# scheckmedia/centernet-uda

Measured on AMD Instinct MI355X. Metric: images/sec CenterNet DLA-34 512x512 UDA step (entropy minimisation), higher is better.
Workload: dtype f32; 1 GPU; configs[2]: DLA-34 + DCNv2, 512x512, per-GPU batch 16 source + 16 target, uda=entropy_minimization, Adam(lr 5e-5), random-init weights; global_batch=16, parallelism=dp1

## Files before the change

centernet-uda_amd/backends/dla.py:

```python
import logging
import math
import os
import warnings

import torch
from torch import nn

from hip_runtime import nn as hnn
from hip_runtime import ops
from hip_runtime.fanout import fork
from libs.DCNv2.dcn_v2 import DCN

log = logging.getLogger(__name__)
PRETRAINED_FILE = 'dla34-ba72cf86.pth'

BN_MOMENTUM = 0.1
DLA34_LEVELS = (1, 1, 1, 2, 2, 1)
DLA34_CHANNELS = (16, 32, 64, 128, 256, 512)


def _bn(c):
    return hnn.BatchNorm2d(c, momentum=BN_MOMENTUM)


_FOLD_GEN = [0]


def _fold_stamp(module):
    import hip_runtime as hr
    if not hasattr(module, '_fold_token'):
        module._fold_token = hr.PackToken()
    _FOLD_GEN[0] += 1
    module._fold_gen = _FOLD_GEN[0]


def _folded(conv_weight, conv_bias, bn):
    with torch.no_grad():
        scale = bn.weight / torch.sqrt(bn.running_var + bn.eps)
        w = (conv_weight * scale.view(-1, 1, 1, 1)).contiguous()
        b = bn.bias - bn.running_mean * scale
        if conv_bias is not None:
            b = b + conv_bias * scale
        return w, b.contiguous()


_FOLDED_INFERENCE = False


class folded_inference:

    def __enter__(self):
        global _FOLDED_INFERENCE
        self.prev, _FOLDED_INFERENCE = _FOLDED_INFERENCE, True

    def __exit__(self, *exc):
        global _FOLDED_INFERENCE
        _FOLDED_INFERENCE = self.prev


def _use_folded(module):
    return (_FOLDED_INFERENCE and getattr(module, '_fold', None) is not None and not module.training
            and not torch.is_grad_enabled())


def fold_batchnorm(model):
    n = 0
    for m in model.modules():
        if hasattr(m, 'fold_batchnorm_'):
            m.fold_batchnorm_()
            n += 1
    return n


def unfold_batchnorm(model):
    for m in model.modules():
        if hasattr(m, 'fold_batchnorm_'):
            m._fold = None


def _conv(cin, cout, k, stride=1):
    return hnn.Conv2d(cin, cout, k, stride=stride, padding=k // 2, bias=False, emit_stats=True)


def _norm_on_load_ok(cin, cout, k):
    try:
        import hip_runtime as hr
        return bool(hr.lib().cnuda_conv2d_norm_input_supported(1, cin, 64, 64, cout, k, k, 1, 1, k // 2, k // 2))
    except Exception:
        return False


class ConvBnRelu(nn.Sequential):

    _fold = None

    def __init__(self, cin, cout, k, stride=1):
        super().__init__(_conv(cin, cout, k, stride), _bn(cout))

    def fold_batchnorm_(self):
        self._fold = _folded(self[0].weight, self[0].bias, self[1])
        _fold_stamp(self)

    def forward(self, x):
        if _use_folded(self):
            return ops.conv2d_infer(x, *self._fold, self[0].stride, self[0].padding, 0.0, None, self._fold_token,
                                    self._fold_gen)
        return self[1](self[0](x), relu=True)


class ConvBn(nn.Sequential):
    _fold = None

    def __init__(self, cin, cout):
        super().__init__(_conv(cin, cout, 1), _bn(cout))

    def fold_batchnorm_(self):
        self._fold = _folded(self[0].weight, self[0].bias, self[1])
        _fold_stamp(self)

    def forward(self, x):
        if _use_folded(self):
            return ops.conv2d_infer(x, *self._fold, self[0].stride, self[0].padding, -1.0, None, self._fold_token,
                                    self._fold_gen)
        return self[1](self[0](x))


class BasicBlock(nn.Module):
    def __init__(self, cin, cout, stride=1):
        super().__init__()
        self.conv1, self.bn1 = _conv(cin, cout, 3, stride), _bn(cout)
        self.conv2, self.bn2 = _conv(cout, cout, 3), _bn(cout)

    _fold = None

    def fold_batchnorm_(self):
        import hip_runtime as hr
        self._fold = _folded(self.conv1.weight, None, self.bn1) + _folded(self.conv2.weight, None, self.bn2)
        _fold_stamp(self)
        if not hasattr(self, '_fold_token2'):
            self._fold_token2 = hr.PackToken()

    def forward(self, x, residual=None):
        if _use_folded(self):
            w1, b1, w2, b2 = self._fold
            y = ops.conv2d_infer(x, w1, b1, self.conv1.stride, self.conv1.padding, 0.0, None, self._fold_token,
                                 self._fold_gen)
            return ops.conv2d_infer(y, w2, b2, 1, 1, 0.0, x if residual is None else residual, self._fold_token2,
                                    self._fold_gen)
        if residual is None or residual is x:
            x, residual = fork(x, 2)
        y = self.bn1(self.conv1(x), relu=True)
        return self.bn2(self.conv2(y), residual=residual, relu=True)


CAT_FREE_ROOT = os.environ.get('CNUDA_CAT_FREE_ROOT', '1') != '0'


class Root(nn.Module):
    def __init__(self, cin, cout):
        super().__init__()
        self.conv, self.bn = _conv(cin, cout, 1), _bn(cout)

    _fold = None

    def fold_batchnorm_(self):
        self._fold = _folded(self.conv.weight, None, self.bn)
        _fold_stamp(self)

    def forward(self, *xs):
        if _use_folded(self):
            y = ops.conv1x1_cat_infer(xs, *self._fold, 0.0, self._fold_token, self._fold_gen) if CAT_FREE_ROOT else None
            return y if y is not None else ops.conv2d_infer(ops.cat_channels(xs), *self._fold, 1, 0, 0.0, None,
                                                            self._fold_token, self._fold_gen)
        y = ops.conv1x1_cat(xs, self.conv.weight, self.conv._pack_token, emit_stats=self.conv.emit_stats and self.training) \
            if CAT_FREE_ROOT and self.conv.kernel_size == (1, 1) and self.conv.bias is None else None
        if y is None:
            y = self.conv(ops.cat_channels(xs))
        return self.bn(y, relu=True)


class Tree(nn.Module):

    def __init__(self, levels, cin, cout, stride=1, level_root=False, root_dim=0):
        super().__init__()
        self.levels, self.level_root = levels, level_root
        root_dim = root_dim or 2 * cout
        if level_root:
            root_dim += cin
        if levels == 1:
            self.tree1 = BasicBlock(cin, cout, stride)
            self.tree2 = BasicBlock(cout, cout, 1)
            self.root = Root(root_dim, cout)
        else:
            self.tree1 = Tree(levels - 1, cin, cout, stride)
            self.tree2 = Tree(levels - 1, cout, cout, root_dim=root_dim + cout)
        self.downsample = hnn.MaxPool2d(stride) if stride > 1 else None
        self.project = ConvBn(cin, cout) if cin != cout else None

    def forward(self, x, children=None):
        children = [] if children is None else children
        if self.downsample is not None:
            x_pool, x = fork(x, 2)
            bottom = self.downsample(x_pool)
            takers = int(self.project is not None or self.levels == 1) + int(self.level_root)
            bs = list(fork(bottom, takers)) if takers > 1 else [bottom]
            residual = self.project(bs.pop()) if self.project is not None else (bs.pop() if self.levels == 1 else None)
            if self.level_root:
                children.append(bs.pop())
        else:
            takers = 1 + int(self.project is not None) + int(self.level_root)
            xs = list(fork(x, takers)) if takers > 1 else [x]
            x = xs.pop()
            residual = self.project(xs.pop()) if self.project is not None else x
            if self.level_root:
                children.append(xs.pop())
        if self.levels == 1:
            x1 = self.tree1(x, residual)
            x1_next, x1_root = fork(x1, 2)
            x2 = self.tree2(x1_next)
            return self.root(x2, x1_root, *children)
        x1 = self.tree1(x)
        x1_next, x1_root = fork(x1, 2)
        children.append(x1_root)
        return self.tree2(x1_next, children=children)


class DLA(nn.Module):
    def __init__(self, levels=DLA34_LEVELS, channels=DLA34_CHANNELS):
        super().__init__()
        c = self.channels = list(channels)
        self.base_layer = ConvBnRelu(3, c[0], 7)
        self.level0 = ConvBnRelu(c[0], c[0], 3)
        self.base_layer[1].defer_apply = _norm_on_load_ok(c[0], c[0], 3)
# ... 292 lines not shown
```

centernet-uda_amd/csrc/conv.hip:

```cpp
#include <stdlib.h>

#include <type_traits>
#include <algorithm>
#include "igemm.cuh"
#include "hconv.cuh"
#include "hwgrad.cuh"
#include "igemm_host.h"

namespace cnuda {
namespace {

struct ConvGeom {
    int B, C, H, W, Co, kh, kw, sh, sw, ph, pw, Ho, Wo;
};

struct ConvFwdParams {
    ConvGeom g;
    const float *x, *bias;
    float* y;
    float act_slope;
    const float* residual;
};
struct ConvFwdStatsParams : ConvFwdParams {
    float* stats;
    int stats_mp;
};

struct ConvFwdSigParams : ConvFwdParams {
    int sig_from;
};
__device__ __forceinline__ float conv_row_sigmoid(float v) { return 1.0f / (1.0f + expf(-v)); }

template <bool FAST>
struct ConvFwdLoader {
    using Params = ConvFwdParams;
    static const char* name() { return FAST ? "ConvFwdLoader<true>" : "ConvFwdLoader<false>"; }
    static constexpr bool kHasSideOutput = false;
    const ConvGeom& g;
    const float* x_b;
    int iy0, ix0;
    bool valid;
    int ck0 = 0, ctap = 0, cc0 = 0, cr = 0, cs = 0;
    __device__ __forceinline__ void seek(int k0) {
        while (ck0 < k0) {
            ck0 += IG_BK;
            cc0 += IG_BK;
            if (cc0 >= g.C) { cc0 -= g.C; ++ctap; if (++cs == g.kw) { cs = 0; ++cr; } }
        }
    }
    __device__ ConvFwdLoader(const Params& p, long long n, bool n_valid) : g(p.g), valid(n_valid) {
        const int HoWo = g.Ho * g.Wo;
        const int nn = n_valid ? (int)n : 0;
        const int b = nn / HoWo, pp = nn - b * HoWo;
        const int oy = pp / g.Wo, ox = pp - oy * g.Wo;
        iy0 = oy * g.sh - g.ph;
        ix0 = ox * g.sw - g.pw;
        x_b = p.x + (size_t)b * g.C * g.H * g.W;
    }
    __device__ __forceinline__ void load(int k0, int ksub, float (&v)[8]) {
        const int HW = g.H * g.W, K = g.kh * g.kw * g.C;
        if (FAST) {
            seek(k0);
            const int c0 = cc0 + ksub;
            const int iy = iy0 + cr, ix = ix0 + cs;
            const bool ok = valid && k0 < K && iy >= 0 && iy < g.H && ix >= 0 && ix < g.W;
            const float* ptr = x_b + (size_t)c0 * HW + (ok ? iy * g.W + ix : 0);
#pragma unroll
            for (int j = 0; j < 8; ++j) v[j] = ok ? ptr[(size_t)(2 * j) * HW] : 0.0f;
        } else {
#pragma unroll
            for (int j = 0; j < 8; ++j) {
                const int k = k0 + ksub + 2 * j;
                float val = 0.0f;
                if (valid && k < K) {
                    const int tap = k / g.C, c = k - tap * g.C;
                    const int r = tap / g.kw, s = tap - r * g.kw;
                    const int iy = iy0 + r, ix = ix0 + s;
                    if (iy >= 0 && iy < g.H && ix >= 0 && ix < g.W) val = x_b[(size_t)c * HW + iy * g.W + ix];
                }
                v[j] = val;
            }
        }
    }
    struct Out {
        float* base;
        const float* res;
        int HoWo;
        __device__ Out(const Params& p, long long n) {
            HoWo = p.g.Ho * p.g.Wo;
            const int ni = (int)n, b = ni / HoWo, pp = ni - b * HoWo;
            base = p.y + (size_t)b * p.g.Co * HoWo + pp;
            res = p.residual ? p.residual + (size_t)b * p.g.Co * HoWo + pp : nullptr;
        }
        __device__ __forceinline__ void store(const Params& p, int m, float v) {
            if (p.bias) v += p.bias[m];
            if (res) v += res[(size_t)m * HoWo];
            if (p.act_slope >= 0.0f && v < 0.0f) v *= p.act_slope;
            base[(size_t)m * HoWo] = v;
        }
        static constexpr bool kVec4 = true;
        __device__ static bool vec4_ok(const Params& p) { return ((p.g.Ho * p.g.Wo) & 3) == 0; }
        __device__ __forceinline__ void store4(const Params& p, int m, f32x4 v) {
            if (p.bias) v += p.bias[m];
            if (res) v += *reinterpret_cast<const f32x4*>(res + (size_t)m * HoWo);
            if (p.act_slope >= 0.0f) {
#pragma unroll
                for (int e = 0; e < 4; ++e) if (v[e] < 0.0f) v[e] *= p.act_slope;
            }
            *reinterpret_cast<f32x4*>(base + (size_t)m * HoWo) = v;
        }
    };
};

struct ConvFwdBufLoader {
    using Params = ConvFwdParams;
    static const char* name() { return "ConvFwdBufLoader"; }
    static constexpr bool kHasSideOutput = false;
    const ConvGeom& g;
    buf_rsrc rs;
    unsigned pix_off;
    unsigned tap_ok;
    int ck0 = 0, ctap = 0, cc0 = 0, cr = 0, cs = 0;
    __device__ __forceinline__ void seek(int k0) {
        while (ck0 < k0) {
            ck0 += IG_BK;
            cc0 += IG_BK;
            if (cc0 >= g.C) { cc0 -= g.C; ++ctap; if (++cs == g.kw) { cs = 0; ++cr; } }
        }
    }
    __device__ ConvFwdBufLoader(const Params& p, long long n, bool n_valid) : g(p.g) {
        const int HoWo = g.Ho * g.Wo;
        const int nn = n_valid ? (int)n : 0;
        const int b = nn / HoWo, pp = nn - b * HoWo;
        const int oy = pp / g.Wo, ox = pp - oy * g.Wo;
        const int iy0 = oy * g.sh - g.ph, ix0 = ox * g.sw - g.pw;
        rs = ig_make_rsrc(p.x, (unsigned)((size_t)g.B * g.C * g.H * g.W * sizeof(float)));
        pix_off = (unsigned)(((b * g.C * g.H + iy0) * g.W + ix0) * (int)sizeof(float));
        tap_ok = 0;
        if (n_valid) {
            for (int r = 0; r < g.kh; ++r)
                for (int s = 0; s < g.kw; ++s) {
                    const int iy = iy0 + r, ix = ix0 + s;
                    if (iy >= 0 && iy < g.H && ix >= 0 && ix < g.W) tap_ok |= 1u << (r * g.kw + s);
                }
        }
    }
    __device__ __forceinline__ void load(int k0, int ksub, float (&v)[8]) {
        const int HW = g.H * g.W;
        seek(k0);
        const int tap = ctap < 32 ? ctap : 31;
        const bool in_k = k0 < g.kh * g.kw * g.C;
        const unsigned voff = (in_k && ((tap_ok >> tap) & 1u)) ? pix_off + (unsigned)((cr * g.W + cs) * (int)sizeof(float))
                                                                : IG_BUF_OOB;
        const int c0 = cc0 + __builtin_amdgcn_readfirstlane(ksub);
#pragma unroll
        for (int j = 0; j < 8; ++j) v[j] = ig_buf_load(rs, voff, (unsigned)((c0 + 2 * j) * HW) * (unsigned)sizeof(float));
    }
    using Out = ConvFwdLoader<true>::Out;
};

struct ConvFwdBufSigLoader : ConvFwdBufLoader {
    using Params = ConvFwdSigParams;
    static const char* name() { return "ConvFwdBufSigLoader"; }
    __device__ ConvFwdBufSigLoader(const Params& p, long long n, bool n_valid) : ConvFwdBufLoader(p, n, n_valid) {}
    struct Out : ConvFwdLoader<true>::Out {
        __device__ Out(const Params& p, long long n) : ConvFwdLoader<true>::Out(p, n) {}
        __device__ __forceinline__ void store(const Params& p, int m, float v) {
            if (p.bias) v += p.bias[m];
            if (m >= p.sig_from) v = conv_row_sigmoid(v);
            base[(size_t)m * HoWo] = v;
        }
        __device__ __forceinline__ void store4(const Params& p, int m, f32x4 v) {
            if (p.bias) v += p.bias[m];
            if (m >= p.sig_from) {
#pragma unroll
                for (int e = 0; e < 4; ++e) v[e] = conv_row_sigmoid(v[e]);
            }
            *reinterpret_cast<f32x4*>(base + (size_t)m * HoWo) = v;
        }
    };
};

struct ConvFwdBufQuadLoader : ConvFwdBufLoader {
    static const char* name() { return "ConvFwdBufQuadLoader"; }
    __device__ ConvFwdBufQuadLoader(const Params& p, long long n, bool n_valid) : ConvFwdBufLoader(p, n, n_valid) {}
    struct Out {
        float* base;
        size_t quad_stride;
        __device__ Out(const Params& p, long long n) {
            const int HoWo = p.g.Ho * p.g.Wo;
            const int ni = (int)n, b = ni / HoWo, pp = ni - b * HoWo;
            base = p.y + (size_t)b * p.g.Co * HoWo + (size_t)pp * 4;
            quad_stride = (size_t)HoWo * 4;
        }
        __device__ __forceinline__ void store(const Params&, int m, float v) { base[(size_t)(m >> 2) * quad_stride + (m & 3)] = v; }
        static constexpr bool kVec4 = false;
        __device__ static bool vec4_ok(const Params&) { return false; }
        static constexpr bool kQuads = true;
        __device__ __forceinline__ void store_quad(const Params&, int m, f32x4 v) {
            *reinterpret_cast<f32x4*>(base + (size_t)(m >> 2) * quad_stride) = v;
        }
    };
};

struct ConvFwdBufStatsLoader : ConvFwdBufLoader {
    using Params = ConvFwdStatsParams;
    static const char* name() { return "ConvFwdBufStatsLoader"; }
    __device__ ConvFwdBufStatsLoader(const Params& p, long long n, bool n_valid) : ConvFwdBufLoader(p, n, n_valid) {}
};

constexpr int CAT_MAX = 4;
struct ConvCat {
    const float* x[CAT_MAX];
    int c[CAT_MAX];
    int k0[CAT_MAX + 1];
    int n;
};
struct ConvFwdCatParams : ConvFwdStatsParams {
    ConvCat cat;
};
struct ConvFwdCatLoader {
    using Params = ConvFwdCatParams;
    static const char* name() { return "ConvFwdCatLoader"; }
    static constexpr bool kHasSideOutput = false;
    const Params& p;
    unsigned pix;
    int b;
    bool valid;
    int ck0 = 0, src = 0, cc0 = 0;
    __device__ ConvFwdCatLoader(const Params& pp, long long n, bool n_valid) : p(pp), valid(n_valid) {
        const int HW = p.g.H * p.g.W;
        const int nn = n_valid ? (int)n : 0;
        b = nn / HW;
        pix = (unsigned)(nn - b * HW) * 4u;
    }
    __device__ __forceinline__ void load(int k0, int ksub, float (&v)[8]) {
        const int HW = p.g.H * p.g.W;
        while (ck0 < k0) {
            ck0 += IG_BK;
            cc0 += IG_BK;
            if (src < p.cat.n && cc0 >= p.cat.c[src]) { cc0 = 0; ++src; }
        }
        const bool in_k = src < p.cat.n;
        const int s = in_k ? src : 0, cs = p.cat.c[s];
        const buf_rsrc rs = ig_make_rsrc(p.cat.x[s], (unsigned)((size_t)p.g.B * cs * HW * sizeof(float)));
        const unsigned voff = (valid && in_k) ? (unsigned)(b * cs * HW) * 4u + pix : IG_BUF_OOB;
        const int c0 = cc0 + __builtin_amdgcn_readfirstlane(ksub);
#pragma unroll
        for (int j = 0; j < 8; ++j) v[j] = ig_buf_load(rs, voff, (unsigned)((c0 + 2 * j) * HW) * (unsigned)sizeof(float));
    }
    using Out = ConvFwdLoader<true>::Out;
};

struct ConvDgradParams {
    ConvGeom g;
    const float* gy;
    float* gx;
    int cop;
    const float* add = nullptr;
    const float* add2 = nullptr;
};
struct ConvDgradLoader {
    using Params = ConvDgradParams;
    static const char* name() { return "ConvDgradLoader"; }
    static constexpr bool kHasSideOutput = false;
    const ConvGeom& g;
    const float* gy_b;
// ... 217 lines not shown
            const int ni = (int)n, b = ni / HcWc, q = ni - b * HcWc;
            const int qy = q / p.Wc, qx = q - qy * p.Wc;
            const size_t o = (size_t)b * p.g.C * HW + (size_t)(p.py + qy * p.g.sh) * p.g.W + p.px + qx * p.g.sw;
            base = p.gx + o;
            addb = p.add ? p.add + o : nullptr;
            addc = p.add2 ? p.add2 + o : nullptr;
        }
        __device__ __forceinline__ void store(const Params&, int m, float v) {
            if (addb) v += addb[(size_t)m * HW];
            if (addc) v += addc[(size_t)m * HW];
            base[(size_t)m * HW] = v;
        }
        static constexpr bool kVec4 = false;
        __device__ static bool vec4_ok(const Params&) { return false; }
        __device__ __forceinline__ void store4(const Params&, int, f32x4) {}
    };
};

struct ConvDgradClassBufLoader {
    using Params = ConvDgradClassParams;
    static const char* name() { return "ConvDgradClassBufLoader"; }
    static constexpr bool kHasSideOutput = false;
    const Params& p;
    buf_rsrc rs;
    unsigned pix_off, tap_ok;
    int ck0 = 0, cti = 0, co0 = 0;
    __device__ ConvDgradClassBufLoader(const Params& pp, long long n, bool n_valid) : p(pp) {
        const ConvGeom& g = p.g;
        const int HcWc = p.Hc * p.Wc;
        const int nn = n_valid ? (int)n : 0;
        const int b = nn / HcWc, q = nn - b * HcWc;
        const int qy = q / p.Wc, qx = q - qy * p.Wc;
        rs = ig_make_rsrc(p.gy, (unsigned)((size_t)g.B * g.Co * g.Ho * g.Wo * sizeof(float)));
        pix_off = (unsigned)(((b * g.Co * g.Ho + qy) * g.Wo + qx) * (int)sizeof(float));
        tap_ok = 0;
        if (n_valid) {
            for (int t = 0; t < p.ntaps; ++t) {
                const int oy = qy + p.tap_dy[t], ox = qx + p.tap_dx[t];
                if (oy >= 0 && oy < g.Ho && ox >= 0 && ox < g.Wo) tap_ok |= 1u << t;
            }
        }
    }
    __device__ __forceinline__ void load(int k0, int ksub, float (&v)[8]) {
        const ConvGeom& g = p.g;
        const int HoWo = g.Ho * g.Wo;
        while (ck0 < k0) {
            ck0 += IG_BK;
            co0 += IG_BK;
            if (co0 >= g.Co) { co0 -= g.Co; ++cti; }
        }
        const int ti = cti < p.ntaps ? cti : 0;
        const int tapoff = p.tap_dy[ti] * g.Wo + p.tap_dx[ti];
        const unsigned voff = (cti < p.ntaps && ((tap_ok >> ti) & 1u)) ? pix_off + (unsigned)(tapoff * (int)sizeof(float))
                                                                        : IG_BUF_OOB;
        const int o0 = co0 + __builtin_amdgcn_readfirstlane(ksub);
#pragma unroll
        for (int j = 0; j < 8; ++j) v[j] = ig_buf_load(rs, voff, (unsigned)((o0 + 2 * j) * HoWo) * (unsigned)sizeof(float));
    }
    using Out = ConvDgradClassLoader::Out;
};

constexpr int MAX_CLASSES = 4;
struct ConvDgradClassSet {
    ConvDgradClassParams cls[MAX_CLASSES];
    const float* A[MAX_CLASSES];
    int Kp[MAX_CLASSES];
};
template <int BM>
__global__ __launch_bounds__(2 * IG_THREADS, (BM == 128 ? 2 : 1)) void igemm_fwd_ws_classes_kernel(
    ConvDgradClassSet s, int Mp, int M, long long N, int n_tiles, int m_tiles) {
    const int c = blockIdx.y;
    igemm_fwd_ws_body<BM, ConvDgradClassBufLoader, IG_KC>(s.cls[c], s.A[c], Mp, s.Kp[c], M, N, n_tiles, m_tiles);
}
template <int BM>
__global__ __launch_bounds__(IG_THREADS, (BM == 128 ? 3 : 1)) void igemm_fwd_classes_kernel(
    ConvDgradClassSet s, int Mp, int M, long long N, int n_tiles, int m_tiles) {
    const int c = blockIdx.y;
    igemm_fwd_body<BM, ConvDgradClassBufLoader>(s.cls[c], s.A[c], Mp, s.Kp[c], M, N, n_tiles, m_tiles);
}

struct ConvWParams {
    ConvGeom g;
    const float *x, *gy;
};
template <int MODE>
struct ConvWLoader {
    using Params = ConvWParams;
    static const char* name() { return MODE == 2 ? "ConvWLoader<2>" : (MODE == 1 ? "ConvWLoader<1>" : "ConvWLoader<0>"); }
    const Params& p;
    IgPixelCursor c;
    __device__ ConvWLoader(const Params& pp, long long n, long long n_end) : p(pp) {
        c.init(n, n_end, p.g.Ho * p.g.Wo, p.g.Wo);
    }
    __device__ __forceinline__ void advance() { c.advance(p.g.Ho * p.g.Wo, p.g.Wo); }
    template <int NV, int STEP>
    __device__ __forceinline__ void load_g(int m0, int msub, float (&v)[NV]) {
        const ConvGeom& g = p.g;
        const int HoWo = g.Ho * g.Wo;
        const float* base = p.gy + (size_t)c.b_ * g.Co * HoWo + c.pp_;
#pragma unroll
        for (int i = 0; i < NV; ++i) {
            const int m = m0 + msub + STEP * i;
            v[i] = (c.valid_ && m < g.Co) ? base[(size_t)m * HoWo] : 0.0f;
        }
    }
    template <int NV, int STEP>
    __device__ __forceinline__ void load_b(int j0, int jsub, float (&v)[NV]) {
        const ConvGeom& g = p.g;
        const int HW = g.H * g.W, K = g.kh * g.kw * g.C;
        const int iy0 = c.oy_ * g.sh - g.ph, ix0 = c.ox_ * g.sw - g.pw;
        const float* x_b = p.x + (size_t)c.b_ * g.C * HW;
        if (MODE == 2) {
            constexpr int PER = 64 / STEP;
#pragma unroll
            for (int h = 0; h < NV / PER; ++h) {
                const int jg = j0 + 64 * h;
                const int tap = jg / g.C, c0 = jg - tap * g.C + jsub;
                const int r = tap / g.kw, s = tap - r * g.kw;
                const int iy = iy0 + r, ix = ix0 + s;
                const bool ok1 = c.valid_ && jg < K && iy >= 0 && iy < g.H && ix >= 0 && ix < g.W;
                const float* ptr = x_b + (size_t)c0 * HW + (ok1 ? iy * g.W + ix : 0);
#pragma unroll
                for (int i = 0; i < PER; ++i) v[PER * h + i] = ok1 ? ptr[(size_t)(STEP * i) * HW] : 0.0f;
            }
            return;
        }
        int cur = -1, off = 0;
        bool ok = false;
#pragma unroll
        for (int i = 0; i < NV; ++i) {
            const int k = j0 + jsub + STEP * i;
            float val = 0.0f;
            if (c.valid_ && k < K) {
                const int tap = k / g.C, ch = k - tap * g.C;
                if (tap != cur) {
                    const int r = tap / g.kw, s = tap - r * g.kw;
                    const int iy = iy0 + r, ix = ix0 + s;
                    ok = iy >= 0 && iy < g.H && ix >= 0 && ix < g.W;
                    off = iy * g.W + ix;
                    cur = tap;
                }
                if (ok) val = x_b[(size_t)ch * HW + off];
            }
            v[i] = val;
        }
    }
};

struct ConvWBufLoader {
    using Params = ConvWParams;
    static const char* name() { return "ConvWBufLoader"; }
    const Params& p;
    buf_rsrc rg, rx;
    IgPixelCursor c;
    unsigned gimg, ximg;
    __device__ ConvWBufLoader(const Params& pp, long long n, long long n_end) : p(pp) {
        const ConvGeom& g = p.g;
        rg = ig_make_rsrc(p.gy, (unsigned)((size_t)g.B * g.Co * g.Ho * g.Wo * sizeof(float)));
        rx = ig_make_rsrc(p.x, (unsigned)((size_t)g.B * g.C * g.H * g.W * sizeof(float)));
        c.init(n, n_end, g.Ho * g.Wo, g.Wo);
        gimg = (unsigned)(c.b_ * g.Co * g.Ho * g.Wo) * 4u;
        ximg = (unsigned)(c.b_ * g.C * g.H * g.W) * 4u;
    }
    __device__ __forceinline__ void advance() {
        const ConvGeom& g = p.g;
        c.advance(g.Ho * g.Wo, g.Wo);
        if (c.crossed_) {
            gimg += (unsigned)(c.crossed_ * g.Co * g.Ho * g.Wo) * 4u;
            ximg += (unsigned)(c.crossed_ * g.C * g.H * g.W) * 4u;
        }
    }
    template <int NV, int STEP>
    __device__ __forceinline__ void load_g(int m0, int msub, float (&v)[NV]) {
        ig_buf_rows<NV, STEP>(rg, c, gimg, p.g.Ho * p.g.Wo, m0, msub, v);
    }
    template <int NV, int STEP>
    __device__ __forceinline__ void load_b(int j0, int jsub, float (&v)[NV]) {
        const ConvGeom& g = p.g;
        const int HW = g.H * g.W, K = g.kh * g.kw * g.C;
        const int iy0 = ig_mad24(c.oy_, g.sh, -g.ph), ix0 = ig_mad24(c.ox_, g.sw, -g.pw);
        const unsigned corner = ximg + (unsigned)(ig_mad24(jsub, HW, ig_mad24(iy0, g.W, ix0))) * 4u;
        constexpr int PER = 64 / STEP;
#pragma unroll
        for (int h = 0; h < NV / PER; ++h) {
            const int jg = j0 + 64 * h;
            const int tap = jg / g.C, c0 = jg - tap * g.C;
            const int r = tap / g.kw, s = tap - r * g.kw;
            const int iy = iy0 + r, ix = ix0 + s;
            const bool ok = c.valid_ && jg < K && (unsigned)iy < (unsigned)g.H && (unsigned)ix < (unsigned)g.W;
            const unsigned voff = ok ? corner + (unsigned)((r * g.W + s) * (int)sizeof(float)) : IG_BUF_OOB;
#pragma unroll
            for (int i = 0; i < PER; ++i)
                v[PER * h + i] = ig_buf_load(rx, voff, (unsigned)((c0 + STEP * i) * HW) * (unsigned)sizeof(float));
        }
    }
};

struct ConvWBufLoaderC8 : ConvWBufLoader {
    static const char* name() { return "ConvWBufLoaderC8"; }
    __device__ ConvWBufLoaderC8(const Params& pp, long long n, long long n_end) : ConvWBufLoader(pp, n, n_end) {}
    template <int NV, int STEP>
    __device__ __forceinline__ void load_b(int j0, int jsub, float (&v)[NV]) {
        static_assert(STEP == 8, "eight row phases: a phase's channels stay inside one tap when 8 | C");
        const ConvGeom& g = p.g;
        const int HW = g.H * g.W, K = g.kh * g.kw * g.C;
        const int iy0 = ig_mad24(c.oy_, g.sh, -g.ph), ix0 = ig_mad24(c.ox_, g.sw, -g.pw);
        const unsigned corner = ximg + (unsigned)(ig_mad24(jsub, HW, ig_mad24(iy0, g.W, ix0))) * 4u;
#pragma unroll
        for (int i = 0; i < NV; ++i) {
            const int jg = j0 + STEP * i;
            const int tap = jg / g.C, c0 = jg - tap * g.C;
            const int r = tap / g.kw, s = tap - r * g.kw;
            const int iy = iy0 + r, ix = ix0 + s;
            const bool ok = c.valid_ && jg < K && (unsigned)iy < (unsigned)g.H && (unsigned)ix < (unsigned)g.W;
            const unsigned voff = ok ? corner + (unsigned)((r * g.W + s) * (int)sizeof(float)) : IG_BUF_OOB;
            v[i] = ig_buf_load(rx, voff, (unsigned)(c0 * HW) * (unsigned)sizeof(float));
        }
    }
};

struct ConvWCatParams : ConvWParams {
    ConvCat cat;
};
struct ConvWCatLoader {
    using Params = ConvWCatParams;
    static const char* name() { return "ConvWCatLoader"; }
    const Params& p;
    buf_rsrc rg;
    IgPixelCursor c;
    unsigned gimg;
    __device__ ConvWCatLoader(const Params& pp, long long n, long long n_end) : p(pp) {
        const ConvGeom& g = p.g;
        rg = ig_make_rsrc(p.gy, (unsigned)((size_t)g.B * g.Co * g.Ho * g.Wo * sizeof(float)));
        c.init(n, n_end, g.Ho * g.Wo, g.Wo);
        gimg = (unsigned)(c.b_ * g.Co * g.Ho * g.Wo) * 4u;
    }
    __device__ __forceinline__ void advance() {
        const ConvGeom& g = p.g;
        c.advance(g.Ho * g.Wo, g.Wo);
        if (c.crossed_) gimg += (unsigned)(c.crossed_ * g.Co * g.Ho * g.Wo) * 4u;
    }
    template <int NV, int STEP>
    __device__ __forceinline__ void load_g(int m0, int msub, float (&v)[NV]) {
        ig_buf_rows<NV, STEP>(rg, c, gimg, p.g.Ho * p.g.Wo, m0, msub, v);
    }
    template <int NV, int STEP>
    __device__ __forceinline__ void load_b(int j0, int jsub, float (&v)[NV]) {
        const ConvGeom& g = p.g;
        const int HW = g.H * g.W;
        constexpr int PER = 64 / STEP;
#pragma unroll
        for (int h = 0; h < NV / PER; ++h) {
            const int jg = j0 + 64 * h;
            int s = 0;
#pragma unroll
            for (int i = 1; i < CAT_MAX; ++i) s += (i < p.cat.n && jg >= p.cat.k0[i]) ? 1 : 0;
            const int cs = p.cat.c[s], c0 = jg - p.cat.k0[s];
            const buf_rsrc rx = ig_make_rsrc(p.cat.x[s], (unsigned)((size_t)g.B * cs * HW * sizeof(float)));
            const bool ok = c.valid_ && jg < g.C;
            const unsigned voff = ok ? (unsigned)(ig_mad24(c.b_, cs, jsub) * HW + c.pp_) * 4u : IG_BUF_OOB;
#pragma unroll
            for (int i = 0; i < PER; ++i)
                v[PER * h + i] = ig_buf_load(rx, voff, (unsigned)((c0 + STEP * i) * HW) * (unsigned)sizeof(float));
        }
    }
};

int fill_geom(ConvGeom& g, int B, int C, int H, int W, int Co, int kh, int kw, int sh, int sw, int ph, int pw,
              const char* who) {
    CNUDA_REQUIRE(B > 0 && C > 0 && H > 0 && W > 0 && Co > 0, "%s: empty tensor", who);
    CNUDA_REQUIRE(kh > 0 && kw > 0 && sh > 0 && sw > 0 && ph >= 0 && pw >= 0, "%s: bad kernel geometry", who);
    g = ConvGeom{B, C, H, W, Co, kh, kw, sh, sw, ph, pw, (H + 2 * ph - kh) / sh + 1, (W + 2 * pw - kw) / sw + 1};
    CNUDA_REQUIRE(H + 2 * ph >= kh && W + 2 * pw >= kw && g.Ho > 0 && g.Wo > 0, "%s: kernel larger than padded input",
                  who);
    return 0;
}

bool wgrad_buffer_ok(const ConvGeom& g) {
    return buffer_addressing() && (size_t)g.B * g.C * g.H * g.W * sizeof(float) < IG_BUF_OOB &&
           (size_t)g.B * g.Co * g.Ho * g.Wo * sizeof(float) < IG_BUF_OOB && (long long)g.H * g.W < (1 << 23) &&
           (long long)g.Ho * g.Wo < (1 << 23);
}
// ... 123 lines not shown
    const long long z = wgrad_splits(tiles, q.wbm, q.wbj, (q.Nf + WG_BP - 1) / WG_BP);
    q.pix_per_split = ((q.Nf + z - 1) / z + WG_BP - 1) / WG_BP * WG_BP;
    q.Z = (int)((q.Nf + q.pix_per_split - 1) / q.pix_per_split);
    q.hw = hwgrad_ok(g);
    q.hw_s2 = !q.hw && hwgrad_s2_ok(g);
    q.hw_tiles = q.hw_tiles_per_split = 0;
    if (q.hw || q.hw_s2) {
        q.hw_tiles = q.hw ? g.B * hwgrad_tiles_y(g) * (g.W / halo_tile_width(g.W)) : g.B * g.Ho * (round_up(g.Wo, HS_BN) / HS_BN);
        const int groups = (g.C / 16) * (q.hw_s2 ? (g.Co + 31) / 32 : 1);
        int zz = std::max(1, 512 / groups);
        if (zz > q.hw_tiles) zz = q.hw_tiles;
        q.hw_tiles_per_split = (q.hw_tiles + zz - 1) / zz;
        q.Z = (q.hw_tiles + q.hw_tiles_per_split - 1) / q.hw_tiles_per_split;
    }
    q.fwd_bytes = carve_bytes(ig_a_bytes(q.Kpf, q.Mpf), 1) + carve_bytes(splitk_slab_bytes(q.skf, g.Co, q.Nf), 1) + 256;
    q.dgrad_bytes = carve_bytes(ig_a_bytes(q.Kpd, q.Mpd), 1) + carve_bytes(splitk_slab_bytes(q.skd, g.C, q.Nd), 1) + 256;
    if (g.sh > 1 || g.sw > 1) {
        const long long Nc = q.Nd / (g.sh * g.sw);
        const int Kpc = round_up(ceil_div(g.kh, g.sh) * ceil_div(g.kw, g.sw) * g.Co, IG_KC);
        const SplitK sc = pick_splitk(g.C, Nc, Kpc);
        const int mp = round_up(g.C, sc.on() ? sc.bm : 32);
        const size_t need = (size_t)g.sh * g.sw * carve_bytes(ig_a_bytes(Kpc, std::max(round_up(g.C, 128), std::max(mp, q.Mpd))), 1) +
                            carve_bytes(splitk_slab_bytes(sc, g.C, Nc), 1) + 256;
        if (need > q.dgrad_bytes) q.dgrad_bytes = need;
    }
    q.wgrad_bytes = carve_bytes((size_t)q.Z * q.Mpw * q.Jp, 4) +
                    carve_bytes(std::max((size_t)g.Co * g.B, (size_t)q.Z * q.Mpw), 4) + 256;

    q.fwd_gemm = q.skf.on() ? FwdPath::BufSplitK
               : hconv_ok(g, g.C, q.bmf) ? FwdPath::Halo
               : q.fwd_buf ? FwdPath::Buf
               : g.C % IG_BK == 0 ? FwdPath::PtrFast : FwdPath::Ptr;
    q.fwd = smallc_supported(g.C, g.Co, g.kh, g.kw, g.sh, g.sw) ? FwdPath::SmallC : q.fwd_gemm;

    if (g.C == 16 && g.kh == 3 && g.kw == 3 && g.sh == 2 && g.sw == 2 && g.ph == 1 && g.pw == 1 && g.Co <= 256 &&
        matrix_mode() == 0 && (size_t)g.Co * 144 * sizeof(float) <= ig_a_bytes(q.Kpd, q.Mpd)) {
        q.dgrad_gemm = DgradPath::S2C16;
    } else if ((g.sh > 1 || g.sw > 1) && g.H % g.sh == 0 && g.W % g.sw == 0 && g.Co % IG_BK == 0 &&
               ceil_div(g.kh, g.sh) * ceil_div(g.kw, g.sw) <= 9) {
        const long long Nc = (long long)g.B * (g.H / g.sh) * (g.W / g.sw);
        bool any_split = false;
        for (int py = 0; py < g.sh && q.dgrad_buf && !any_split; ++py)
            for (int px = 0; px < g.sw && !any_split; ++px) {
                int ntaps = 0;
                for (int r = 0; r < g.kh; ++r)
                    for (int t = 0; t < g.kw; ++t) ntaps += class_tap(g, py, px, r, t);
                any_split = pick_splitk(g.C, Nc, class_kp(ntaps, g.Co)).on();
            }
        q.dgrad_gemm = (q.dgrad_buf && !any_split && g.sh * g.sw <= MAX_CLASSES && matrix_mode() == 0) ? DgradPath::Classes
                                                                                                    : DgradPath::ClassLoop;
    } else {
        q.dgrad_gemm = q.skd.on() ? DgradPath::BufSplitK
                     : hconv_ok(g, g.Co, q.bmd) ? DgradPath::Halo
                     : (q.dgrad_buf && g.sh == 1 && g.sw == 1) ? DgradPath::Buf : DgradPath::Ptr;
    }
    q.dgrad = (g.sh == 1 && g.sw == 1 && smallc_supported(g.Co, g.C, g.kh, g.kw, 1, 1) && g.kh - 1 - g.ph >= 0 && g.kw - 1 - g.pw >= 0)
                  ? DgradPath::SmallC : q.dgrad_gemm;

    const bool fast = g.C % 64 == 0;
    q.wgrad = smallc_supported(g.C, g.Co, g.kh, g.kw, g.sh, g.sw) ? WgradPath::SmallC
            : q.hw_s2 ? WgradPath::HaloS2
            : q.hw ? WgradPath::Halo
            : (!fast && g.C % 8 == 0 && wbuf && (q.wbm == 32 || (q.wbm == 64 && q.wbj == 64))) ? WgradPath::BufC8
            : (fast && wbuf) ? WgradPath::Buf
            : (fast && wave_specialised() && q.wbm == 64) ? WgradPath::PtrFastWs
            : fast ? WgradPath::PtrFast : WgradPath::Ptr;
    q.wgrad_ws = wave_specialised() && q.wbm >= 64 && (q.wgrad == WgradPath::Buf || q.wgrad == WgradPath::PtrFastWs);
    q.max_bytes = std::max(q.fwd_bytes, std::max(q.dgrad_bytes, q.wgrad_bytes));
    if (q.fwd == FwdPath::SmallC || smallc_supported(g.Co, g.C, g.kh, g.kw, g.sh, g.sw))
        q.max_bytes = std::max(q.max_bytes, smallc_workspace_bytes(g.B, g.C, g.H, g.W, g.Co, g.kh, g.kw, g.sh, g.ph, g.pw) +
                                                carve_bytes((size_t)g.Co * g.B, 4));
    return q;
}

int plan_stats_block(const ConvGeom& g, const ConvPlan& q, int* rows, int* blocks_per_image) {
    if (blocks_per_image) *blocks_per_image = 0;
    if (q.fwd == FwdPath::SmallC)
        return smallc_stats_blocks(g.B, g.C, g.H, g.W, g.Co, g.kh, g.kw, g.sh, g.ph, g.pw, blocks_per_image, rows);
    if (q.fwd != FwdPath::Buf || ((g.Ho * g.Wo) & 3) != 0 || matrix_mode() != 0) return 0;
    if (rows) *rows = q.Mpf;
    return q.bmf == 32 ? 32 : 64;
}

struct HconvFwd {
    using Params = ConvFwdParams;
    using Out = ConvFwdLoader<true>::Out;
    static const char* name() { return "fwd"; }
};
struct HconvFwdSig {
    using Params = ConvFwdSigParams;
    using Out = ConvFwdBufSigLoader::Out;
    static const char* name() { return "fwd, row sigmoid"; }
};
struct HconvDgrad {
    using Params = ConvDgradParams;
    using Out = ConvDgradLoader::Out;
    static const char* name() { return "dgrad"; }
};
template <int BM, int BN, class Ad>
bool hconv_launch_one(const typename Ad::Params& p, const float* src, const float* A, int Mp, int Kp, int M, long long N,
                      int m_tiles, const HaloGeom& hg, hipStream_t st) {
    const size_t lds = hconv_lds_bytes(hg, BM);
    if (!raise_dynamic_lds(reinterpret_cast<const void*>(&hconv_kernel<BM, BN, Ad>), lds)) return false;
    const int n_tiles = (int)(N / ((long long)hg.H * hg.W)) * hg.tiles_y * hg.tiles_x;
    CNUDA_LAUNCH((hconv_kernel<BM, BN, Ad>), dim3(n_tiles * m_tiles), dim3(IG_THREADS), lds, st, p, src, A, Mp, Kp, M, N,
                 n_tiles, m_tiles, hg);
    return true;
}
template <class Ad>
int launch_hconv(int bm, const typename Ad::Params& p, const float* src, int kc, const ConvGeom& g, const float* A, int Mp,
                 int Kp, int M, long long N, hipStream_t st, const char* who) {
    CNUDA_REQUIRE(N < (1ll << 31) - 256, "%s: more than 2^31 pixels per call", who);
    const int m_tiles = Mp / bm;
    const HaloGeom hg2 = make_halo_geom(kc, g.H, g.W, 256);
    const bool wide = bm <= 64 && hg2.TW >= 32 && g.H % hg2.TR == 0 && hg2.cells <= HC_MAXCELLS * IG_THREADS &&
                      (N / 256) * m_tiles >= 1024;
    const HaloGeom hg = wide ? hg2 : make_halo_geom(kc, g.H, g.W, 128);
    ProfScope prof(st);
    prof.name("hconv_kernel<%d, %d, %s>", bm, wide ? 256 : 128, Ad::name());
    bool ok = false;
    CNUDA_REQUIRE((with_tiles<Tile<128, 128>, Tile<64, 256>, Tile<64, 128>, Tile<32, 256>, Tile<32, 128>>(
                      bm, wide ? 256 : 128, [&](auto BM, auto BN) {
                          ok = hconv_launch_one<BM(), BN(), Ad>(p, src, A, Mp, Kp, M, N, m_tiles, hg, st);
                      })),
                  "%s: no hconv_kernel instance for a %d-row tile", who, bm);
    if (!ok) return CNUDA_ERR_INVALID_ARGUMENT;
    return check_launch(who);
}

struct DgradS2Params {
    const float *gy, *wt;
    float* gx;
    const float *add, *add2;
    int B, Co, H, W, Ho, Wo, QH, QW;
};
__global__ __launch_bounds__(256) void dgrad_s2_c16_pack_kernel(const float* __restrict__ w, float* __restrict__ wt, int Co) {
    const int i = blockIdx.x * 256 + threadIdx.x;
    if (i < Co * 144) {
        const int c = i & 15, t = (i >> 4) % 9, o = i / 144;
        wt[i] = w[(o * 16 + c) * 9 + t];
    }
}
__global__ __launch_bounds__(256) void dgrad_s2_c16_kernel(DgradS2Params p) {
    const int qx = blockIdx.x * 64 + (threadIdx.x & 63);
    const int qy = blockIdx.y * 4 + (threadIdx.x >> 6);
    const int b = blockIdx.z;
    if (qy >= p.QH) return;
    const int HoWo = p.Ho * p.Wo, HW = p.H * p.W;
    const bool x0 = qx < p.Wo, x1 = qx + 1 < p.Wo, y0 = qy < p.Ho, y1 = qy + 1 < p.Ho;
    const float* g00 = p.gy + (size_t)b * p.Co * HoWo + (size_t)(y0 ? qy : 0) * p.Wo + (x0 ? qx : 0);
    const int d01 = x1 ? 1 : 0, d10 = y1 ? p.Wo : 0;
    float acc[4][16];
#pragma unroll
    for (int q = 0; q < 4; ++q)
#pragma unroll
        for (int c = 0; c < 16; ++c) acc[q][c] = 0.0f;
    for (int o = 0; o < p.Co; ++o) {
        const float* gp = g00 + (size_t)o * HoWo;
        float a = gp[0], bb = gp[d01], cc = gp[d10], dd = gp[d10 + d01];
        if (!(x0 && y0)) a = 0.0f;
        if (!(x1 && y0)) bb = 0.0f;
        if (!(x0 && y1)) cc = 0.0f;
        if (!(x1 && y1)) dd = 0.0f;
        const float* wo = p.wt + (size_t)o * 144;
#pragma unroll
        for (int c = 0; c < 16; ++c) {
// ... 38 lines not shown
template <class Loader>
int launch_fwd(int bm, const typename Loader::Params& p, const float* A, int Mp, int Kp, int M, long long N,
               hipStream_t st, const char* who, const SplitK& sk = SplitK(), float* slab = nullptr) {
    CNUDA_REQUIRE(N < (1ll << 31) - IG_BN, "%s: more than 2^31 pixels per call", who);
    const int n_tiles = ceil_div(N, IG_BN), m_tiles = Mp / bm;
    const dim3 grid(n_tiles * m_tiles), block(IG_THREADS), block2(2 * IG_THREADS);
    const bool ws = matrix_mode() == 0 && wave_specialised() && bm >= 64;
    bool found;
    ProfScope prof(st);
    if constexpr (SplitKLoader<Loader>::value) {
        if (sk.on()) {
            CNUDA_REQUIRE(slab && bm == sk.bm && matrix_mode() == 0, "%s: split-K plan without its slabs", who);
            prof.name(ws ? "igemm_fwd_ws_splitk_kernel<%d, %s> x %d + reduce" : "igemm_fwd_splitk_kernel<%d, %s> x %d + reduce",
                      bm, Loader::name(), sk.z);
            const dim3 gridz(n_tiles * m_tiles, sk.z);
            if (ws)
                found = with_tile<64, 128>(bm, [&](auto BM) {
                    CNUDA_LAUNCH((igemm_fwd_ws_splitk_kernel<BM(), Loader>), gridz, block2, 0, st, p, A, Mp, Kp, M, N, n_tiles, m_tiles, slab, sk.split_k);
                });
            else
                found = with_tile<32, 64, 128>(bm, [&](auto BM) {
                    CNUDA_LAUNCH((igemm_fwd_splitk_kernel<BM(), Loader>), gridz, block, 0, st, p, A, Mp, Kp, M, N, n_tiles, m_tiles, slab, sk.split_k);
                });
            CNUDA_REQUIRE(found, "%s: no split-K kernel instance for a %d-row tile", who, bm);
            CNUDA_LAUNCH((splitk_reduce_kernel<Loader>), dim3(ceil_div(N, 256), ceil_div(M, SK_ROWS)), dim3(256), 0, st, p, slab, sk.z,
                         Mp, (long long)n_tiles * IG_BN, M, N);
            return check_launch(who);
        }
    }
    CNUDA_REQUIRE(!sk.on(), "%s: split-K plan for a loader without split-K kernels", who);
    if constexpr (std::is_same<Loader, ConvFwdBufLoader>::value || std::is_same<Loader, ConvFwdBufStatsLoader>::value ||
                  std::is_same<Loader, ConvFwdLoader<true>>::value || std::is_same<Loader, ConvFwdBufQuadLoader>::value) {
        static const bool shortk = !(getenv("CNUDA_SHORTK") && getenv("CNUDA_SHORTK")[0] == '0');
        if (shortk && matrix_mode() == 0 && bm == 128 && Kp <= 64 && m_tiles >= 2) {
            prof.name("igemm_fwd_shortk_kernel<128, %s, 64>", Loader::name());
            CNUDA_LAUNCH((igemm_fwd_shortk_kernel<128, Loader, 64>), dim3(n_tiles), block, 0, st, p, A, Mp, Kp, M, N,
                               n_tiles, m_tiles);
            return check_launch(who);
        }
    }
    prof.name(matrix_mode() == 1 ? "igemm_fwd_kernel<%d, %s> [split bf16 x3]"
                                 : (ws ? "igemm_fwd_ws_kernel<%d, %s>" : "igemm_fwd_kernel<%d, %s>"), bm, Loader::name());
    if (matrix_mode() == 1) {
        float* A3 = const_cast<float*>(A) + (size_t)Kp * Mp;
        CNUDA_LAUNCH(split_a_kernel, dim3(stream_grid((long long)(Kp / 16) * 2 * Mp, 256)), dim3(256), 0, st, A,
                           reinterpret_cast<u32x4*>(A3), Kp, Mp);
        found = with_tile<32, 64, 128>(bm, [&](auto BM) {
            CNUDA_LAUNCH((igemm_fwd_kernel<BM(), Loader, true>), grid, block, 0, st, p, A3, Mp, Kp, M, N, n_tiles, m_tiles);
        });
    } else if (ws) {
        found = with_tile<64, 128>(bm, [&](auto BM) {
            CNUDA_LAUNCH((igemm_fwd_ws_kernel<BM(), Loader>), grid, block2, 0, st, p, A, Mp, Kp, M, N, n_tiles, m_tiles);
        });
    } else {
        found = with_tile<32, 64, 128>(bm, [&](auto BM) {
            CNUDA_LAUNCH((igemm_fwd_kernel<BM(), Loader>), grid, block, 0, st, p, A, Mp, Kp, M, N, n_tiles, m_tiles);
        });
    }
    CNUDA_REQUIRE(found, "%s: no igemm_fwd kernel instance for a %d-row tile", who, bm);
    return check_launch(who);
}

template <class Loader, bool WS, class... Tiles, class P>
bool launch_wgrad(const ConvPlan& q, const P& p, float* slabs, float* bsl, hipStream_t st) {
    const dim3 grid(q.Jp / q.wbj, q.Mpw / q.wbm, q.Z), blk((WS ? 2 : 1) * IG_THREADS);
    return with_tiles<Tiles...>(q.wbm, q.wbj, [&](auto BM, auto BJ) {
        if constexpr (WS)
            CNUDA_LAUNCH((igemm_wgrad_ws_kernel<Loader, BM(), BJ()>), grid, blk, 0, st, p, slabs, q.Mpw, q.Jp, q.Nf, q.pix_per_split, bsl);
        else
            CNUDA_LAUNCH((igemm_wgrad_kernel<Loader, BM(), BJ()>), grid, blk, 0, st, p, slabs, q.Mpw, q.Jp, q.Nf, q.pix_per_split, bsl);
    });
}
template <class Loader>
bool launch_wgrad_buf(const ConvPlan& q, const typename Loader::Params& p, float* slabs, float* bsl, hipStream_t st) {
    return q.wgrad_ws ? launch_wgrad<Loader, true, Tile<128, 128>, Tile<128, 64>, Tile<64, 128>, Tile<64, 64>>(q, p, slabs, bsl, st)
                      : launch_wgrad<Loader, false, Tile<128, 128>, Tile<128, 64>, Tile<64, 128>, Tile<64, 64>, Tile<32, 128>>(q, p, slabs, bsl, st);
}

}
}

using namespace cnuda;


extern "C" int cnuda_conv_set_splitk_policy(int max_tiles) {
    const int prev = g_splitk_max_tiles;
    g_splitk_max_tiles = max_tiles < 0 ? 128 : max_tiles;
    return prev;
}

extern "C" int cnuda_conv_set_halo_policy(int level, int min_tiles) {
    if (level >= 0) g_hconv_level = level;
    if (min_tiles >= 1) g_hconv_min_tiles = min_tiles;
    return g_hconv_level | (g_hconv_min_tiles << 8);
}

extern "C" size_t cnuda_conv2d_workspace_bytes(int B, int C, int H, int W, int Cout, int kh, int kw, int sh, int sw,
                                               int ph, int pw) {
    ConvGeom g;
    if (fill_geom(g, B, C, H, W, Cout, kh, kw, sh, sw, ph, pw, "cnuda_conv2d_workspace_bytes")) return 0;
    return make_plan(g).max_bytes;
}

extern "C" int cnuda_conv2d_forward(const float* x, const float* weight, const float* bias, float* y, int B, int C,
                                    int H, int W, int Cout, int kh, int kw, int sh, int sw, int ph, int pw, float act_slope,
                                    void* workspace, size_t workspace_bytes, cnuda_stream_t stream) {
    return cnuda_conv2d_forward_res(x, weight, bias, nullptr, y, B, C, H, W, Cout, kh, kw, sh, sw, ph, pw, act_slope,
                                    workspace, workspace_bytes, stream);
}

extern "C" int cnuda_conv2d_stats_block(int B, int C, int H, int W, int Cout, int kh, int kw, int sh, int sw, int ph,
                                        int pw, int* rows, int* blocks_per_image) {
    ConvGeom g;
    if (fill_geom(g, B, C, H, W, Cout, kh, kw, sh, sw, ph, pw, "cnuda_conv2d_stats_block")) return 0;
    return plan_stats_block(g, make_plan(g), rows, blocks_per_image);
}

extern "C" int cnuda_conv2d_forward_res(const float* x, const float* weight, const float* bias, const float* residual,
                                        float* y, int B, int C, int H, int W, int Cout, int kh, int kw, int sh, int sw,
                                        int ph, int pw, float act_slope, void* workspace, size_t workspace_bytes,
                                        cnuda_stream_t stream) {
    return cnuda_conv2d_forward_stats(x, weight, bias, residual, y, nullptr, B, C, H, W, Cout, kh, kw, sh, sw, ph, pw, act_slope,
                                      workspace, workspace_bytes, stream);
}

extern "C" int cnuda_conv2d_forward_stats(const float* x, const float* weight, const float* bias, const float* residual,
                                          float* y, float* stats, int B, int C, int H, int W, int Cout, int kh, int kw,
                                          int sh, int sw, int ph, int pw, float act_slope, void* workspace,
                                          size_t workspace_bytes, cnuda_stream_t stream) {
    CNUDA_REQUIRE(x && weight && y, "cnuda_conv2d_forward: null pointer");
    ConvGeom g;
    if (int rc = fill_geom(g, B, C, H, W, Cout, kh, kw, sh, sw, ph, pw, "cnuda_conv2d_forward")) return rc;
    const ConvPlan q = make_plan(g);
    CNUDA_REQUIRE(!stats || (!residual && act_slope < 0.0f && plan_stats_block(g, q, nullptr, nullptr) != 0),
                  "cnuda_conv2d_forward_stats: no statistics for this call (cnuda_conv2d_stats_block says which)");
    const FwdPath path = residual ? q.fwd_gemm : q.fwd;
    if (path == FwdPath::SmallC)
        return smallc_forward(x, weight, bias, y, B, C, H, W, Cout, kh, kw, sh, ph, pw, act_slope, 0, workspace,
                              workspace_bytes, (hipStream_t)stream, stats);
    CNUDA_REQUIRE(workspace && workspace_bytes >= q.fwd_bytes, "cnuda_conv2d_forward: workspace too small");
    hipStream_t st = (hipStream_t)stream;
    Carver cv(workspace, workspace_bytes);
    ConvFwdParams p{g, x, bias, y, act_slope, residual};
    const float* A = launch_pack(weight, reinterpret_cast<float*>(cv.take<char>(ig_a_bytes(q.Kpf, q.Mpf))), ig_a_bytes(q.Kpf, q.Mpf),
                                 Cout, C, q.T, path == FwdPath::Halo ? PACK_HALO_FWD : PACK_FWD, q.Kpf, q.Mpf, 0, st);
    switch (path) {
        case FwdPath::Halo:
            return launch_hconv<HconvFwd>(q.bmf, p, x, C, g, A, q.Mpf, q.Kpf, Cout, q.Nf, st, "cnuda_conv2d_forward");
        case FwdPath::BufSplitK: {
            float* slab = reinterpret_cast<float*>(cv.take<char>(splitk_slab_bytes(q.skf, Cout, q.Nf)));
            return launch_fwd<ConvFwdBufLoader>(q.bmf, p, A, q.Mpf, q.Kpf, Cout, q.Nf, st, "cnuda_conv2d_forward", q.skf, slab);
        }
        case FwdPath::Buf:
            if (stats) {
                ConvFwdStatsParams ps;
                static_cast<ConvFwdParams&>(ps) = p;
                ps.stats = stats;
                ps.stats_mp = q.Mpf;
                return launch_fwd<ConvFwdBufStatsLoader>(q.bmf, ps, A, q.Mpf, q.Kpf, Cout, q.Nf, st, "cnuda_conv2d_forward_stats");
            }
            return launch_fwd<ConvFwdBufLoader>(q.bmf, p, A, q.Mpf, q.Kpf, Cout, q.Nf, st, "cnuda_conv2d_forward");
        case FwdPath::PtrFast:
            return launch_fwd<ConvFwdLoader<true>>(q.bmf, p, A, q.Mpf, q.Kpf, Cout, q.Nf, st, "cnuda_conv2d_forward");
        default:
            return launch_fwd<ConvFwdLoader<false>>(q.bmf, p, A, q.Mpf, q.Kpf, Cout, q.Nf, st, "cnuda_conv2d_forward");
    }
}

namespace {
int fill_cat(ConvCat& cat, const float* const* xs, const int* cs, int n, const char* who) {
    CNUDA_REQUIRE(xs && cs && n >= 2 && n <= CAT_MAX, "%s: 2 .. %d sources", who, CAT_MAX);
    int k = 0;
    for (int i = 0; i < CAT_MAX; ++i) {
        cat.x[i] = i < n ? xs[i] : nullptr;
        cat.c[i] = i < n ? cs[i] : 0;
        cat.k0[i] = k;
        if (i < n) {
            CNUDA_REQUIRE(xs[i] && cs[i] > 0 && cs[i] % 64 == 0, "%s: source %d: null or not a multiple of 64 channels", who, i);
            k += cs[i];
        }
    }
    cat.k0[CAT_MAX] = k;
    for (int i = n; i < CAT_MAX; ++i) cat.k0[i] = k;
    cat.n = n;
    return 0;
}
int cat_channels(const int* cs, int n) {
    int k = 0;
    for (int i = 0; i < n; ++i) k += cs[i];
    return k;
}
}

extern "C" int cnuda_conv2d_cat_supported(const int* cs, int n, int B, int H, int W, int Cout) {
    if (!cs || n < 2 || n > CAT_MAX || matrix_mode() != 0) return 0;
    for (int i = 0; i < n; ++i)
        if (cs[i] <= 0 || cs[i] % 64 != 0) return 0;
    const int C = cat_channels(cs, n);
    ConvGeom g;
    if (fill_geom(g, B, C, H, W, Cout, 1, 1, 1, 1, 0, 0, "cnuda_conv2d_cat_supported")) return 0;
    const ConvPlan q = make_plan(g);
    return q.fwd == FwdPath::Buf && q.dgrad == DgradPath::Buf && q.wgrad == WgradPath::Buf && ((H * W) & 3) == 0;
}

extern "C" int cnuda_conv2d_cat_forward(const float* const* xs, const int* cs, int n, const float* weight, const float* bias,
                                        float* y, float* stats, float act_slope, int B, int H, int W, int Cout,
                                        void* workspace, size_t workspace_bytes, cnuda_stream_t stream) {
    CNUDA_REQUIRE(weight && y, "cnuda_conv2d_cat_forward: null pointer");
    CNUDA_REQUIRE(!stats || act_slope < 0.0f, "cnuda_conv2d_cat_forward: statistics are those of the plain convolution");
    CNUDA_REQUIRE(cnuda_conv2d_cat_supported(cs, n, B, H, W, Cout), "cnuda_conv2d_cat_forward: unsupported (cnuda_conv2d_cat_supported)");
    ConvFwdCatParams p;
    if (int rc = fill_cat(p.cat, xs, cs, n, "cnuda_conv2d_cat_forward")) return rc;
    const int C = p.cat.k0[CAT_MAX];
    ConvGeom g;
    if (int rc = fill_geom(g, B, C, H, W, Cout, 1, 1, 1, 1, 0, 0, "cnuda_conv2d_cat_forward")) return rc;
    const ConvPlan q = make_plan(g);
    CNUDA_REQUIRE(workspace && workspace_bytes >= q.fwd_bytes, "cnuda_conv2d_cat_forward: workspace too small");
    hipStream_t st = (hipStream_t)stream;
    Carver cv(workspace, workspace_bytes);
    static_cast<ConvFwdParams&>(p) = ConvFwdParams{g, nullptr, bias, y, act_slope, nullptr};
    p.stats = stats;
    p.stats_mp = q.Mpf;
    const float* A = launch_pack(weight, reinterpret_cast<float*>(cv.take<char>(ig_a_bytes(q.Kpf, q.Mpf))),
                                 ig_a_bytes(q.Kpf, q.Mpf), Cout, C, q.T, PACK_FWD, q.Kpf, q.Mpf, 0, st);
    return launch_fwd<ConvFwdCatLoader>(q.bmf, p, A, q.Mpf, q.Kpf, Cout, q.Nf, st, "cnuda_conv2d_cat_forward");
}
// ... 39 lines not shown
    ConvGeom g;
    if (int rc = fill_geom(g, B, C, H, W, Cout, 1, 1, 1, 1, 0, 0, "cnuda_conv2d_cat_backward_weight")) return rc;
    const ConvPlan q = make_plan(g);
    CNUDA_REQUIRE(workspace && workspace_bytes >= q.wgrad_bytes, "cnuda_conv2d_cat_backward_weight: workspace too small");
    hipStream_t st = (hipStream_t)stream;
    Carver cv(workspace, workspace_bytes);
    float* slabs = cv.take<float>((size_t)q.Z * q.Mpw * q.Jp);
    static_cast<ConvWParams&>(p) = ConvWParams{g, nullptr, grad_y};
    {
        ProfScope prof(st);
        prof.name(q.wgrad_ws ? "igemm_wgrad_ws_kernel<ConvWCatLoader, %d, %d>" : "igemm_wgrad_kernel<ConvWCatLoader, %d, %d>",
                  q.wbm, q.wbj);
        CNUDA_REQUIRE(launch_wgrad_buf<ConvWCatLoader>(q, p, slabs, nullptr, st),
                      "cnuda_conv2d_cat_backward_weight: no kernel instance for a %d x %d tile", q.wbm, q.wbj);
    }
    if (int rc = check_launch("cnuda_conv2d_cat_backward_weight")) return rc;
    launch_slab_reduce(slabs, grad_weight, q.Z, q.Mpw, q.Jp, Cout, C, q.T, st, nullptr, nullptr);
    return check_launch("cnuda_conv2d_cat_backward_weight(reduce)");
}

extern "C" int cnuda_conv2d_rowquads_supported(int B, int C, int H, int W, int Cout, int kh, int kw, int sh, int sw, int ph,
                                               int pw) {
    ConvGeom g;
    if (fill_geom(g, B, C, H, W, Cout, kh, kw, sh, sw, ph, pw, "cnuda_conv2d_rowquads_supported")) return 0;
    const ConvPlan q = make_plan(g);
    return Cout % 4 == 0 && q.fwd != FwdPath::SmallC && q.fwd != FwdPath::BufSplitK && q.fwd_buf;
}

extern "C" int cnuda_conv2d_forward_rowquads(const float* x, const float* weight, float* y, int B, int C, int H, int W,
                                             int Cout, int kh, int kw, int sh, int sw, int ph, int pw, void* workspace,
                                             size_t workspace_bytes, cnuda_stream_t stream) {
    CNUDA_REQUIRE(x && weight && y, "cnuda_conv2d_forward_rowquads: null pointer");
    CNUDA_REQUIRE(cnuda_conv2d_rowquads_supported(B, C, H, W, Cout, kh, kw, sh, sw, ph, pw),
                  "cnuda_conv2d_forward_rowquads: geometry without a quad-interleaved epilogue (cnuda_conv2d_rowquads_supported)");
    ConvGeom g;
    if (int rc = fill_geom(g, B, C, H, W, Cout, kh, kw, sh, sw, ph, pw, "cnuda_conv2d_forward_rowquads")) return rc;
    const ConvPlan q = make_plan(g);
    CNUDA_REQUIRE(workspace && workspace_bytes >= q.fwd_bytes, "cnuda_conv2d_forward_rowquads: workspace too small");
    hipStream_t st = (hipStream_t)stream;
    Carver cv(workspace, workspace_bytes);
    ConvFwdParams p{g, x, nullptr, y, -1.0f, nullptr};
    const float* A = launch_pack(weight, reinterpret_cast<float*>(cv.take<char>(ig_a_bytes(q.Kpf, q.Mpf))),
                                 ig_a_bytes(q.Kpf, q.Mpf), Cout, C, q.T, PACK_FWD, q.Kpf, q.Mpf, 0, st);
    return launch_fwd<ConvFwdBufQuadLoader>(q.bmf, p, A, q.Mpf, q.Kpf, Cout, q.Nf, st, "cnuda_conv2d_forward_rowquads");
}

extern "C" int cnuda_conv2d_rowsig_supported(int B, int C, int H, int W, int Cout, int kh, int kw, int sh, int sw, int ph,
                                             int pw) {
    ConvGeom g;
    if (fill_geom(g, B, C, H, W, Cout, kh, kw, sh, sw, ph, pw, "cnuda_conv2d_rowsig_supported")) return 0;
    const ConvPlan q = make_plan(g);
    return (Cout <= 32 && matrix_mode() == 0 && q.fwd != FwdPath::SmallC && q.fwd_buf && q.y_buf) ? 1 : 0;
}
extern "C" int cnuda_conv2d_forward_rowsig(const float* x, const float* weight, const float* bias, float* y, int sig_from,
                                           int B, int C, int H, int W, int Cout, int kh, int kw, int sh, int sw, int ph, int pw,
                                           void* workspace, size_t workspace_bytes, cnuda_stream_t stream) {
    CNUDA_REQUIRE(x && weight && y && sig_from >= 0, "cnuda_conv2d_forward_rowsig: bad arguments");
    CNUDA_REQUIRE(cnuda_conv2d_rowsig_supported(B, C, H, W, Cout, kh, kw, sh, sw, ph, pw),
                  "cnuda_conv2d_forward_rowsig: geometry without a row-sigmoid epilogue (cnuda_conv2d_rowsig_supported)");
    ConvGeom g;
    if (int rc = fill_geom(g, B, C, H, W, Cout, kh, kw, sh, sw, ph, pw, "cnuda_conv2d_forward_rowsig")) return rc;
    const ConvPlan q = make_plan(g);
    CNUDA_REQUIRE(workspace && workspace_bytes >= q.fwd_bytes, "cnuda_conv2d_forward_rowsig: workspace too small");
    hipStream_t st = (hipStream_t)stream;
    Carver cv(workspace, workspace_bytes);
    ConvFwdSigParams p;
    static_cast<ConvFwdParams&>(p) = ConvFwdParams{g, x, bias, y, -1.0f, nullptr};
    p.sig_from = sig_from;
    const bool halo = q.fwd == FwdPath::Halo;
    const float* A = launch_pack(weight, reinterpret_cast<float*>(cv.take<char>(ig_a_bytes(q.Kpf, q.Mpf))), ig_a_bytes(q.Kpf, q.Mpf),
                                 Cout, C, q.T, halo ? PACK_HALO_FWD : PACK_FWD, q.Kpf, q.Mpf, 0, st);
    if (halo) return launch_hconv<HconvFwdSig>(q.bmf, p, x, C, g, A, q.Mpf, q.Kpf, Cout, q.Nf, st, "cnuda_conv2d_forward_rowsig");
    float* slab = q.skf.on() ? reinterpret_cast<float*>(cv.take<char>(splitk_slab_bytes(q.skf, Cout, q.Nf))) : nullptr;
    return launch_fwd<ConvFwdBufSigLoader>(q.bmf, p, A, q.Mpf, q.Kpf, Cout, q.Nf, st, "cnuda_conv2d_forward_rowsig", q.skf, slab);
}

extern "C" int cnuda_conv2d_backward_data(const float* grad_y, const float* weight, float* grad_x, int B, int C, int H,
                                          int W, int Cout, int kh, int kw, int sh, int sw, int ph, int pw,
                                          void* workspace, size_t workspace_bytes, cnuda_stream_t stream) {
    return cnuda_conv2d_backward_data_add(grad_y, weight, nullptr, nullptr, grad_x, B, C, H, W, Cout, kh, kw, sh, sw, ph, pw, workspace,
                                          workspace_bytes, stream);
}

extern "C" int cnuda_conv2d_norm_input_supported(int B, int C, int H, int W, int Cout, int kh, int kw, int sh, int sw, int ph,
                                                 int pw) {
    (void)B; (void)H; (void)W;
    return ph == (kh - 1) / 2 && pw == (kw - 1) / 2 && smallc_norm_supported(C, Cout, kh, kw, sh, sw) ? 1 : 0;
}
extern "C" int cnuda_conv2d_forward_norm_input(const float* x, const float* mean, const float* invstd, const float* gamma,
                                               const float* beta, int imgs_per_group, const float* weight, const float* bias,
                                               float* y, float* stats, int B, int C, int H, int W, int Cout, int kh, int kw,
                                               int sh, int sw, int ph, int pw, float act_slope, void* workspace,
                                               size_t workspace_bytes, cnuda_stream_t stream) {
    CNUDA_REQUIRE(x && mean && invstd && gamma && beta && weight && y, "cnuda_conv2d_forward_norm_input: null pointer");
    CNUDA_REQUIRE(imgs_per_group > 0 && B % imgs_per_group == 0, "cnuda_conv2d_forward_norm_input: statistics groups");
    CNUDA_REQUIRE(cnuda_conv2d_norm_input_supported(B, C, H, W, Cout, kh, kw, sh, sw, ph, pw),
                  "cnuda_conv2d_forward_norm_input: geometry without an apply-on-load kernel");
    if (stats) {
        int rows = 0;
        CNUDA_REQUIRE(act_slope < 0.0f && cnuda_conv2d_stats_block(B, C, H, W, Cout, kh, kw, sh, sw, ph, pw, &rows, nullptr) != 0,
                      "cnuda_conv2d_forward_norm_input: no statistics for this call");
    }
    const SmallNorm nm{mean, invstd, gamma, beta, imgs_per_group};
    return smallc_forward(x, weight, bias, y, B, C, H, W, Cout, kh, kw, sh, ph, pw, act_slope, 0, workspace, workspace_bytes,
                          (hipStream_t)stream, stats, &nm);
}
extern "C" int cnuda_conv2d_backward_weight_norm_input(const float* x, const float* mean, const float* invstd,
                                                       const float* gamma, const float* beta, int imgs_per_group,
                                                       const float* grad_y, float* grad_weight, float* grad_bias, int B, int C,
                                                       int H, int W, int Cout, int kh, int kw, int sh, int sw, int ph, int pw,
                                                       void* workspace, size_t workspace_bytes, cnuda_stream_t stream) {
    CNUDA_REQUIRE(x && mean && invstd && gamma && beta && grad_y && grad_weight,
                  "cnuda_conv2d_backward_weight_norm_input: null pointer");
    CNUDA_REQUIRE(imgs_per_group > 0 && B % imgs_per_group == 0, "cnuda_conv2d_backward_weight_norm_input: statistics groups");
    CNUDA_REQUIRE(cnuda_conv2d_norm_input_supported(B, C, H, W, Cout, kh, kw, sh, sw, ph, pw),
                  "cnuda_conv2d_backward_weight_norm_input: geometry without an apply-on-load kernel");
    ConvGeom g;
    if (int rc = fill_geom(g, B, C, H, W, Cout, kh, kw, sh, sw, ph, pw, "cnuda_conv2d_backward_weight_norm_input")) return rc;
    hipStream_t st = (hipStream_t)stream;
    const SmallNorm nm{mean, invstd, gamma, beta, imgs_per_group};
    if (int rc = smallc_backward_weight(x, grad_y, grad_weight, B, C, H, W, Cout, kh, kw, sh, ph, pw, workspace, workspace_bytes,
                                        st, &nm))
        return rc;
    if (grad_bias) launch_channel_sum(grad_y, grad_bias, B, Cout, (long long)g.Ho * g.Wo, st);
    return check_launch("cnuda_conv2d_backward_weight_norm_input");
}

extern "C" int cnuda_conv2d_backward_data_add(const float* grad_y, const float* weight, const float* addend,
                                              const float* addend2, float* grad_x, int B, int C, int H, int W, int Cout,
                                              int kh, int kw, int sh, int sw, int ph, int pw, void* workspace,
                                              size_t workspace_bytes, cnuda_stream_t stream) {
    if (!addend && addend2) { addend = addend2; addend2 = nullptr; }
    CNUDA_REQUIRE(grad_y && weight && grad_x, "cnuda_conv2d_backward_data: null pointer");
    ConvGeom g;
    if (int rc = fill_geom(g, B, C, H, W, Cout, kh, kw, sh, sw, ph, pw, "cnuda_conv2d_backward_data")) return rc;
    const bool aliased = (addend && addend == grad_x) || (addend2 && addend2 == grad_x);
    const ConvPlan q = make_plan(g);
    const DgradPath path = aliased ? q.dgrad_gemm : q.dgrad;
    if (path == DgradPath::SmallC) {
        if (int rc = smallc_forward(grad_y, weight, nullptr, grad_x, B, Cout, g.Ho, g.Wo, C, kh, kw, 1, kh - 1 - ph,
                                    kw - 1 - pw, -1.0f, 1, workspace, workspace_bytes, (hipStream_t)stream))
            return rc;
        if (addend) if (int rc = cnuda_add(grad_x, addend, grad_x, (long long)B * C * H * W, stream)) return rc;
        return addend2 ? cnuda_add(grad_x, addend2, grad_x, (long long)B * C * H * W, stream) : 0;
    }
    CNUDA_REQUIRE(workspace && workspace_bytes >= q.dgrad_bytes, "cnuda_conv2d_backward_data: workspace too small");
    hipStream_t st = (hipStream_t)stream;
    Carver cv(workspace, workspace_bytes);
    float* Aws = reinterpret_cast<float*>(cv.take<char>(ig_a_bytes(q.Kpd, q.Mpd)));
    if (path == DgradPath::S2C16) {
        CNUDA_LAUNCH(dgrad_s2_c16_pack_kernel, dim3((Cout * 144 + 255) / 256), dim3(256), 0, st, weight, Aws, Cout);
        DgradS2Params dp{grad_y, Aws, grad_x, addend, addend2, B, Cout, H, W, g.Ho, g.Wo, (H + 1) / 2, (W + 1) / 2};
        ProfScope prof(st);
        prof.name("dgrad_s2_c16_kernel");
        CNUDA_LAUNCH(dgrad_s2_c16_kernel, dim3((dp.QW + 63) / 64, (dp.QH + 3) / 4, B), dim3(256), 0, st, dp);
        return check_launch("cnuda_conv2d_backward_data(stride 2, 16 channels)");
    }
    if (path == DgradPath::Classes || path == DgradPath::ClassLoop) {
        const bool buf_ok = q.dgrad_buf;
        ProfScope prof(st);
        prof.name("igemm_fwd*_kernel<*, ConvDgradClassLoader> x %d parity classes", sh * sw);
        const long long Nc = (long long)B * (H / sh) * (W / sw);
        ConvDgradClassParams cps[16];
        int Kpcs[16], taps_all[16][9], ncls = 0;
        for (int py = 0; py < sh; ++py)
            for (int px = 0; px < sw; ++px) {
                CNUDA_REQUIRE(ncls < 16, "cnuda_conv2d_backward_data: more than 16 parity classes");
                ConvDgradClassParams& cp = cps[ncls];
                cp.g = g; cp.gy = grad_y; cp.gx = grad_x; cp.py = py; cp.px = px; cp.Hc = H / sh; cp.Wc = W / sw;
                cp.add = addend; cp.add2 = addend2;
                cp.ntaps = 0;
                for (int r = 0; r < kh; ++r)
                    for (int t = 0; t < kw; ++t)
                        if (class_tap(g, py, px, r, t)) {
                            cp.tap_r[cp.ntaps] = r; cp.tap_s[cp.ntaps] = t; taps_all[ncls][cp.ntaps] = r * kw + t;
                            cp.tap_dy[cp.ntaps] = (py + ph - r) / sh; cp.tap_dx[cp.ntaps] = (px + pw - t) / sw;
                            ++cp.ntaps;
                        }
                Kpcs[ncls] = class_kp(cp.ntaps, Cout);
                ++ncls;
            }
        if (path == DgradPath::Classes) {
            const int bm = conv_pick_bm(C, Nc * ncls), Mp = round_up(C, bm);
            int order[MAX_CLASSES];
            for (int i = 0; i < ncls; ++i) order[i] = i;
            std::stable_sort(order, order + ncls, [&](int a, int b2) { return Kpcs[a] > Kpcs[b2]; });
            ConvDgradClassSet set;
            size_t used = 0;
            for (int i = 0; i < ncls; ++i) {
                const int c = order[i];
                const size_t bytes = carve_bytes(ig_a_bytes(Kpcs[c], Mp), 1);
                CNUDA_REQUIRE(used + bytes + 256 <= workspace_bytes, "cnuda_conv2d_backward_data: workspace");
                float* dst = reinterpret_cast<float*>(reinterpret_cast<char*>(Aws) + used);
                used += bytes;
                set.cls[i] = cps[c];
                set.Kp[i] = Kpcs[c];
                set.A[i] = launch_pack_taps(weight, dst, ig_a_bytes(Kpcs[c], Mp), Cout, C, q.T, taps_all[c], cps[c].ntaps, Kpcs[c], Mp, st);
            }
            for (int i = ncls; i < MAX_CLASSES; ++i) { set.cls[i] = set.cls[0]; set.Kp[i] = set.Kp[0]; set.A[i] = set.A[0]; }
            CNUDA_REQUIRE(Nc < (1ll << 31) - IG_BN, "cnuda_conv2d_backward_data: more than 2^31 pixels per call");
            const int n_tiles = ceil_div(Nc, IG_BN), m_tiles = Mp / bm;
            const dim3 grid(n_tiles * m_tiles, ncls);
            const bool found = (wave_specialised() && bm >= 64)
                ? with_tile<64, 128>(bm, [&](auto BM) {
                      CNUDA_LAUNCH((igemm_fwd_ws_classes_kernel<BM()>), grid, dim3(2 * IG_THREADS), 0, st, set, Mp, C, Nc, n_tiles, m_tiles);
                  })
                : with_tile<32, 64, 128>(bm, [&](auto BM) {
                      CNUDA_LAUNCH((igemm_fwd_classes_kernel<BM()>), grid, dim3(IG_THREADS), 0, st, set, Mp, C, Nc, n_tiles, m_tiles);
                  });
            CNUDA_REQUIRE(found, "cnuda_conv2d_backward_data: no parity-class kernel instance for a %d-row tile", bm);
            return check_launch("cnuda_conv2d_backward_data(classes)");
        }
        for (int ci = 0; ci < ncls; ++ci) {
                const ConvDgradClassParams& cp = cps[ci];
                const int Kpc = Kpcs[ci];
                const int* taps = taps_all[ci];
                const SplitK sc = buf_ok ? pick_splitk(C, Nc, Kpc) : SplitK();
                const int bm = sc.on() ? sc.bm : conv_pick_bm(C, Nc), Mp = round_up(C, bm);
                const size_t slab_bytes = splitk_slab_bytes(sc, C, Nc);
                CNUDA_REQUIRE(carve_bytes(ig_a_bytes(Kpc, Mp), 1) + carve_bytes(slab_bytes, 1) + 256 <= workspace_bytes,
                              "cnuda_conv2d_backward_data: workspace");
                const float* A = launch_pack_taps(weight, Aws, ig_a_bytes(Kpc, Mp), Cout, C, q.T, taps, cp.ntaps, Kpc, Mp, st);
                float* slab = sc.on() ? reinterpret_cast<float*>((reinterpret_cast<uintptr_t>(Aws) + ig_a_bytes(Kpc, Mp) + 255) & ~(uintptr_t)255) : nullptr;
                if (int rc = buf_ok ? launch_fwd<ConvDgradClassBufLoader>(bm, cp, A, Mp, Kpc, C, Nc, st, "cnuda_conv2d_backward_data(class)", sc, slab)
                                    : launch_fwd<ConvDgradClassLoader>(bm, cp, A, Mp, Kpc, C, Nc, st, "cnuda_conv2d_backward_data(class)"))
                    return rc;
        }
        return 0;
    }
    if (path == DgradPath::Halo) {
        const float* Ah = launch_pack(weight, Aws, ig_a_bytes(q.Kpd, q.Mpd), Cout, C, q.T, PACK_HALO_DGRAD, q.Kpd, q.Mpd, 0, st);
        ConvDgradParams ph{g, grad_y, grad_x, Cout, addend, addend2};
        return launch_hconv<HconvDgrad>(q.bmd, ph, grad_y, Cout, g, Ah, q.Mpd, q.Kpd, C, q.Nd, st, "cnuda_conv2d_backward_data");
    }
    const float* A = launch_pack(weight, Aws, ig_a_bytes(q.Kpd, q.Mpd), Cout, C, q.T, PACK_DGRAD, q.Kpd, q.Mpd,
                                 round_up(Cout, IG_BK), st);
    ConvDgradParams p{g, grad_y, grad_x, round_up(Cout, IG_BK), addend, addend2};
    if (path == DgradPath::BufSplitK || path == DgradPath::Buf) {
        float* slab = q.skd.on() ? reinterpret_cast<float*>(cv.take<char>(splitk_slab_bytes(q.skd, C, q.Nd))) : nullptr;
        return launch_fwd<ConvDgradBufLoader>(q.bmd, p, A, q.Mpd, q.Kpd, C, q.Nd, st, "cnuda_conv2d_backward_data", q.skd, slab);
    }
    return launch_fwd<ConvDgradLoader>(q.bmd, p, A, q.Mpd, q.Kpd, C, q.Nd, st, "cnuda_conv2d_backward_data");
}

extern "C" int cnuda_conv2d_backward_weight(const float* x, const float* grad_y, float* grad_weight, float* grad_bias,
                                            int B, int C, int H, int W, int Cout, int kh, int kw, int sh, int sw,
                                            int ph, int pw, void* workspace, size_t workspace_bytes,
                                            cnuda_stream_t stream) {
    CNUDA_REQUIRE(x && grad_y && grad_weight, "cnuda_conv2d_backward_weight: null pointer");
    ConvGeom g;
    if (int rc = fill_geom(g, B, C, H, W, Cout, kh, kw, sh, sw, ph, pw, "cnuda_conv2d_backward_weight")) return rc;
    const ConvPlan q = make_plan(g);
    hipStream_t st = (hipStream_t)stream;
    if (q.wgrad == WgradPath::SmallC) {
        if (int rc = smallc_backward_weight(x, grad_y, grad_weight, B, C, H, W, Cout, kh, kw, sh, ph, pw, workspace,
                                            workspace_bytes, st))
            return rc;
        if (grad_bias) launch_channel_sum(grad_y, grad_bias, B, Cout, (long long)g.Ho * g.Wo, st);
        return check_launch("cnuda_conv2d_backward_weight(small)");
    }
    CNUDA_REQUIRE(workspace && workspace_bytes >= q.wgrad_bytes, "cnuda_conv2d_backward_weight: workspace too small");
    Carver cv(workspace, workspace_bytes);
    float* slabs = cv.take<float>((size_t)q.Z * q.Mpw * q.Jp);
    float* bsl = grad_bias ? cv.take<float>((size_t)q.Z * q.Mpw) : nullptr;
    ConvWParams p{g, x, grad_y};
    bool found = true, lds_ok = true;
    {
        ProfScope prof(st);
        if (q.wgrad == WgradPath::HaloS2) {
            prof.name("hwgrad_s2_kernel");
            const HwS2Params hp{x, grad_y, B, C, H, W, Cout, g.Ho, g.Wo, q.hw_tiles, q.hw_tiles_per_split};
            const size_t lds = HS_LDS_FLOATS * sizeof(float);
            lds_ok = raise_dynamic_lds(reinterpret_cast<const void*>(&hwgrad_s2_kernel), lds);
            if (lds_ok)
                CNUDA_LAUNCH(hwgrad_s2_kernel, dim3(C / 16, q.Z, (Cout + 31) / 32), dim3(IG_THREADS), lds, st, hp, slabs, q.Mpw, q.Jp, bsl);
        } else if (q.wgrad == WgradPath::Halo) {
            const int tw = halo_tile_width(W);
            const bool side = tw < W;
            prof.name(side ? "hwgrad_kernel<%d, side>" : "hwgrad_kernel<%d>", tw);
            const HwParams hp{x, grad_y, B, C, H, W, Cout, W / tw, hwgrad_tiles_y(g), q.hw_tiles, q.hw_tiles_per_split};
            found = with_tiles<Tile<128, 0>, Tile<64, 0>, Tile<32, 0>, Tile<16, 0>, Tile<8, 0>,
                               Tile<128, 1>, Tile<64, 1>, Tile<32, 1>, Tile<16, 1>, Tile<8, 1>>(tw, side ? 1 : 0, [&](auto TW, auto SIDE) {
                constexpr bool kSide = SIDE() != 0;
                const size_t lds = HwShape<TW(), kSide>::lds_floats * sizeof(float);
                lds_ok = raise_dynamic_lds(reinterpret_cast<const void*>(&hwgrad_kernel<TW(), kSide>), lds);
                if (lds_ok) CNUDA_LAUNCH((hwgrad_kernel<TW(), kSide>), dim3(C / 16, q.Z), dim3(IG_THREADS), lds, st, hp, slabs, q.Mpw, q.Jp, bsl);
            });
        } else {
            prof.name(q.wgrad_ws ? "igemm_wgrad_ws_kernel<%s, %d, %d>" : "igemm_wgrad_kernel<%s, %d, %d>", wgrad_loader_name(q.wgrad),
                      q.wbm, q.wbj);
            switch (q.wgrad) {
                case WgradPath::BufC8:
                    found = launch_wgrad<ConvWBufLoaderC8, false, Tile<32, 128>, Tile<64, 64>>(q, p, slabs, bsl, st);
                    break;
                case WgradPath::Buf:
                    found = launch_wgrad_buf<ConvWBufLoader>(q, p, slabs, bsl, st);
                    break;
                case WgradPath::PtrFastWs:
                    found = launch_wgrad<ConvWLoader<2>, true, Tile<64, 128>, Tile<64, 64>>(q, p, slabs, bsl, st);
                    break;
                case WgradPath::PtrFast:
                    found = launch_wgrad<ConvWLoader<2>, false, Tile<64, 128>, Tile<64, 64>, Tile<32, 128>>(q, p, slabs, bsl, st);
                    break;
                default:
                    found = launch_wgrad<ConvWLoader<0>, false, Tile<64, 64>, Tile<32, 128>>(q, p, slabs, bsl, st);
            }
        }
    }
    CNUDA_REQUIRE(lds_ok, "cnuda_conv2d_backward_weight: dynamic LDS");
    CNUDA_REQUIRE(found, "cnuda_conv2d_backward_weight: no kernel instance for this tile (%d x %d)", q.wbm, q.wbj);
    if (int rc = check_launch("cnuda_conv2d_backward_weight")) return rc;
    launch_slab_reduce(slabs, grad_weight, q.Z, q.Mpw, q.Jp, Cout, C, q.T, st, bsl, grad_bias);
    return check_launch("cnuda_conv2d_backward_weight(reduce)");
}
```

centernet-uda_amd/csrc/igemm.cuh:

```cuda
#pragma once
#include <type_traits>
#include <utility>
#include "common.h"

namespace cnuda {

using f32x16 = __attribute__((ext_vector_type(16))) float;

constexpr int IG_BN = 128;
constexpr int IG_BK = 16;
constexpr int IG_KC = 16;
constexpr int IG_THREADS = 256;

template <int BM> struct IgTile;
template <> struct IgTile<128> { static constexpr int WM = 2, WN = 2, TM = 2, TN = 2; };
template <> struct IgTile<64>  { static constexpr int WM = 2, WN = 2, TM = 1, TN = 2; };
template <> struct IgTile<32>  { static constexpr int WM = 1, WN = 4, TM = 1, TN = 1; };

__device__ __forceinline__ int xcd_remap(int bid, int nwg) {
    constexpr int NX = 8;
    const int per = nwg / NX, rem = nwg % NX;
    const int x = bid % NX, q = bid / NX;
    const int start = x * per + (x < rem ? x : rem);
    return start + q;
// ... 195 lines not shown
    using T = IgTile<BM>;
    const int col = lane & 31, cg = lane & 7, rsub = lane >> 3;
    constexpr bool kStats = IgHasStats<typename Loader::Params>::value;
    bool stats_on = false;
    if constexpr (kStats) stats_on = p.stats != nullptr;
    float ssum[T::TM][4], ssq[T::TM][4];
#pragma unroll
    for (int i = 0; i < T::TM; ++i)
#pragma unroll
        for (int it = 0; it < 4; ++it) { ssum[i][it] = 0.0f; ssq[i][it] = 0.0f; }
#pragma unroll
    for (int j = 0; j < T::TN; ++j) {
        const long long n = n0 + wn_off + j * 32 + 4 * cg;
        typename Loader::Out out(p, n < N ? n : 0);
#pragma unroll
        for (int i = 0; i < T::TM; ++i) {
#pragma unroll
            for (int r = 0; r < 16; ++r) stage[mfma_row(r, lane) * IG_EPI_LD + col] = acc[i][j][r];
            asm volatile("s_waitcnt lgkmcnt(0)" ::: "memory");
#pragma unroll
            for (int it = 0; it < 4; ++it) {
                const int row = it * 8 + rsub;
                const f32x4 v = *reinterpret_cast<const f32x4*>(stage + row * IG_EPI_LD + 4 * cg);
                const int m = m0 + wm_off + i * 32 + row;
                if (m < M && n < N) out.store4(p, m, v);
                if constexpr (kStats) {
                    if (stats_on) {
                        f32x4 w = v;
                        if (p.bias && m < M) w += p.bias[m];
                        if (!(n < N)) w = f32x4{0.f, 0.f, 0.f, 0.f};
                        ssum[i][it] += (w[0] + w[1]) + (w[2] + w[3]);
                        ssq[i][it] += (w[0] * w[0] + w[1] * w[1]) + (w[2] * w[2] + w[3] * w[3]);
                    }
                }
            }
            asm volatile("s_waitcnt lgkmcnt(0)" ::: "memory");
        }
    }
    if constexpr (kStats) {
        if (stats_on) {
            auto row8 = [](float v) {
                v += __builtin_bit_cast(float, __builtin_amdgcn_update_dpp(0, __builtin_bit_cast(int, v), 0xB1, 0xf, 0xf, false));
                v += __builtin_bit_cast(float, __builtin_amdgcn_update_dpp(0, __builtin_bit_cast(int, v), 0x4E, 0xf, 0xf, false));
                v += __builtin_bit_cast(float, __builtin_amdgcn_update_dpp(0, __builtin_bit_cast(int, v), 0x141, 0xf, 0xf, false));
                return v;
            };
            const long long blk = (n0 + wn_off) / ig_stat_px<BM>();
            float2* dst = reinterpret_cast<float2*>(p.stats) + blk * p.stats_mp + m0 + wm_off;
#pragma unroll
            for (int i = 0; i < T::TM; ++i)
#pragma unroll
                for (int it = 0; it < 4; ++it) {
                    const float a = row8(ssum[i][it]), b = row8(ssq[i][it]);
                    if (cg == 0) dst[i * 32 + it * 8 + rsub] = make_float2(a, b);
                }
        }
    }
}

template <class O, class = void> struct IgHasQuads : std::false_type {};
template <class O> struct IgHasQuads<O, std::void_t<decltype(O::kQuads)>> : std::true_type {};
template <int BM, class Loader>
__device__ __forceinline__ void ig_epilogue_quads(const typename Loader::Params& p,
                                                  const f32x16 (&acc)[IgTile<BM>::TM][IgTile<BM>::TN], int m0, long long n0,
                                                  int wm_off, int wn_off, int lane, int M, long long N) {
    using T = IgTile<BM>;
#pragma unroll
    for (int j = 0; j < T::TN; ++j) {
        const long long n = n0 + wn_off + j * 32 + (lane & 31);
        if (n >= N) continue;
        typename Loader::Out out(p, n);
#pragma unroll
        for (int i = 0; i < T::TM; ++i)
#pragma unroll
            for (int q = 0; q < 4; ++q) {
                const int m = m0 + wm_off + i * 32 + 8 * q + 4 * (lane >> 5);
                if (m < M) out.store_quad(p, m, f32x4{acc[i][j][4 * q], acc[i][j][4 * q + 1], acc[i][j][4 * q + 2], acc[i][j][4 * q + 3]});
            }
    }
}

template <class Loader, bool TWO_PHASE> struct IgRaw { struct type {}; };
template <class Loader> struct IgRaw<Loader, true> { using type = typename Loader::Raw; };

template <int BM>
__device__ __forceinline__ void ig_store_slab(float* __restrict__ slab, const f32x16 (&acc)[IgTile<BM>::TM][IgTile<BM>::TN],
                                              int Mp, long long Np, int m0, long long n0, int wm_off, int wn_off, int lane) {
    using T = IgTile<BM>;
    float* const d = slab + (size_t)blockIdx.y * Mp * Np;
#pragma unroll
    for (int j = 0; j < T::TN; ++j) {
        const long long n = n0 + wn_off + j * 32 + (lane & 31);
#pragma unroll
        for (int i = 0; i < T::TM; ++i)
#pragma unroll
            for (int r = 0; r < 16; ++r) d[(size_t)(m0 + wm_off + i * 32 + mfma_row(r, lane)) * Np + n] = acc[i][j][r];
    }
}

template <int BM, class Loader, bool X3 = false, bool SPLITK = false>
__device__ __forceinline__ void igemm_fwd_body(
    const typename Loader::Params& p, const float* __restrict__ A, int Mp, int Kp, int M, long long N,
    int n_tiles, int m_tiles, float* __restrict__ slab = nullptr, int split_k = 0) {
    using T = IgTile<BM>;
    static_assert(!(X3 && SPLITK), "split-K runs on the f32 pipe");
    constexpr int LDS_A = X3 ? 3 * 2 * BM * 4 : IG_KC * BM, LDS_B = X3 ? 3 * 2 * IG_BN * 4 : IG_KC * IG_BN;
    constexpr int LDS_AB = 2 * LDS_A + 2 * LDS_B;
    static_assert(LDS_AB >= 4 * IG_EPI_WAVE, "the operand buffers hold the epilogue staging tiles");
    __shared__ __attribute__((aligned(16))) float smem[LDS_AB];
    float (*As)[LDS_A] = reinterpret_cast<float (*)[LDS_A]>(smem);
    float (*Bs)[LDS_B] = reinterpret_cast<float (*)[LDS_B]>(smem + 2 * LDS_A);
    const int tid = threadIdx.x, lane = tid & 63, wid = tid >> 6;
    const int wg = xcd_remap(blockIdx.x, n_tiles * m_tiles);
    const int m0 = (wg % m_tiles) * BM;
    const long long n0 = (long long)(wg / m_tiles) * IG_BN;
    const int wm_off = (wid / T::WN) * (T::TM * 32), wn_off = (wid % T::WN) * (T::TN * 32);

    const int nl = tid & (IG_BN - 1), ksub = tid >> 7;
    Loader ld(p, n0 + nl, n0 + nl < N);
    if constexpr (Loader::kHasSideOutput) { if (m0 != 0) ld.disable_col(); }

    f32x16 acc[T::TM][T::TN];
#pragma unroll
    for (int i = 0; i < T::TM; ++i)
#pragma unroll
        for (int j = 0; j < T::TN; ++j)
#pragma unroll
            for (int r = 0; r < 16; ++r) acc[i][j][r] = 0.0f;

    constexpr int NH = IG_KC / IG_BK;
    f32x4 ra[ig_a_per<BM>()];
    float rb[NH][8];
    u32x4 ra3[ig_a3_per<BM>()];
    typename IgRaw<Loader, Loader::kHasSideOutput>::type raw[NH];
    const IgABuf<BM> abuf(A, Mp, Kp, m0, tid);
    auto stage_store = [&](int buf) {
        if constexpr (X3) ig_store_a_x3<BM>(reinterpret_cast<u32x4*>(As[buf]), tid, ra3);
        else ig_store_a<BM>(As[buf], tid, ra);
        if constexpr (Loader::kHasSideOutput) {
#pragma unroll
            for (int h = 0; h < NH; ++h) ld.finish(raw[h], rb[h]);
        }
        if constexpr (X3) {
            static_assert(NH == 1, "X3 stages one 16-deep MFMA step per chunk");
            unsigned o[3][4];
            x3_split<8>(rb[0], o);
#pragma unroll
            for (int pc = 0; pc < 3; ++pc)
                reinterpret_cast<u32x4*>(Bs[buf])[(pc * 2 + ksub) * IG_BN + nl] = u32x4{o[pc][0], o[pc][1], o[pc][2], o[pc][3]};
        } else {
#pragma unroll
            for (int h = 0; h < NH; ++h)
#pragma unroll
                for (int j = 0; j < 8; ++j) Bs[buf][(h * IG_BK + ksub + 2 * j) * IG_BN + nl] = rb[h][j];
        }
    };
    auto stage_load = [&](int k0) {
        if constexpr (X3) ig_load_a_x3<BM>(reinterpret_cast<const u32x4*>(A), Mp, k0, m0, tid, ra3);
        else abuf.load(k0, ra);
#pragma unroll
        for (int h = 0; h < NH; ++h) {
            if constexpr (Loader::kHasSideOutput) ld.load_raw(k0 + h * IG_BK, ksub, raw[h]);
            else ld.load(k0 + h * IG_BK, ksub, rb[h]);
        }
    };
    if constexpr (X3) {
        const int nchunk = Kp / IG_KC, klast = Kp - IG_KC;
        auto kclamp = [&](int c) { const int k = c * IG_KC; return k < klast ? k : klast; };
        auto frag_read = [&](int st, u32x4 (&fa)[T::TM][3], u32x4 (&fb)[T::TN][3]) {
            ig_read_frag_x3<BM>(reinterpret_cast<const u32x4*>(As[st]), reinterpret_cast<const u32x4*>(Bs[st]), fa, fb,
                                wm_off, wn_off, lane);
        };
        u32x4 fa0[T::TM][3], fb0[T::TN][3], fa1[T::TM][3], fb1[T::TN][3];
        stage_load(0);
        stage_store(0);
        stage_load(kclamp(1));
        __syncthreads();
        frag_read(0, fa0, fb0);
        stage_store(1);
        stage_load(kclamp(2));
        __syncthreads();
        auto step = [&](int c, u32x4 (&ca)[T::TM][3], u32x4 (&cb)[T::TN][3], u32x4 (&na)[T::TM][3], u32x4 (&nb)[T::TN][3]) {
            frag_read((c + 1) & 1, na, nb);
            ig_mma_frag_x3<BM>(ca, cb, acc);
            stage_store(c & 1);
#pragma unroll
            for (int i = 0; i < 6 * T::TM * T::TN; ++i) {
                __builtin_amdgcn_sched_group_barrier(0x008, 1, 0);
                __builtin_amdgcn_sched_group_barrier(0x002, BM == 128 ? 3 : (BM == 64 ? 5 : 6), 0);
            }
            stage_load(kclamp(c + 3));
            __syncthreads();
        };
        constexpr int X3_FOLD = 8;
        f32x16 total[T::TM][T::TN];
#pragma unroll
        for (int i = 0; i < T::TM; ++i)
#pragma unroll
            for (int j = 0; j < T::TN; ++j)
#pragma unroll
                for (int r = 0; r < 16; ++r) total[i][j][r] = 0.0f;
        auto fold = [&]() {
#pragma unroll
            for (int i = 0; i < T::TM; ++i)
#pragma unroll
                for (int j = 0; j < T::TN; ++j)
#pragma unroll
                    for (int r = 0; r < 16; ++r) { total[i][j][r] += acc[i][j][r]; acc[i][j][r] = 0.0f; }
        };
        int c = 0;
        for (; c + 1 < nchunk; c += 2) {
            step(c, fa0, fb0, fa1, fb1);
            step(c + 1, fa1, fb1, fa0, fb0);
            if (((c + 2) & (X3_FOLD - 1)) == 0) fold();
        }
        if (c < nchunk) ig_mma_frag_x3<BM>(fa0, fb0, acc);
#pragma unroll
        for (int i = 0; i < T::TM; ++i)
#pragma unroll
            for (int j = 0; j < T::TN; ++j)
#pragma unroll
                for (int r = 0; r < 16; ++r) acc[i][j][r] += total[i][j][r];
    } else {
    const int kb = SPLITK ? (int)blockIdx.y * split_k : 0;
// ... 6 lines not shown
    for (int k0 = kb; k0 < ke; k0 += IG_KC) {
        ig_mma_chunk<BM>(As[cur], Bs[cur], acc, wm_off, wn_off, lane);
        if (k0 + IG_KC < ke) {
            stage_store(cur ^ 1);
            if (k0 + 2 * IG_KC < ke) stage_load(k0 + 2 * IG_KC);
        }
        __syncthreads();
        cur ^= 1;
    }
    }
    if constexpr (SPLITK) {
        ig_store_slab<BM>(slab, acc, Mp, (long long)n_tiles * IG_BN, m0, n0, wm_off, wn_off, lane);
        return;
    }
    if constexpr (IgHasQuads<typename Loader::Out>::value) {
        ig_epilogue_quads<BM, Loader>(p, acc, m0, n0, wm_off, wn_off, lane, M, N);
        return;
    }
    if constexpr (Loader::Out::kVec4) {
        if (Loader::Out::vec4_ok(p)) {
            ig_epilogue_vec4<BM, Loader>(p, smem + wid * IG_EPI_WAVE, acc, m0, n0, wm_off, wn_off, lane, M, N);
            return;
        }
    }
#pragma unroll
    for (int j = 0; j < T::TN; ++j) {
        const long long n = n0 + wn_off + j * 32 + (lane & 31);
        if (n >= N) continue;
        typename Loader::Out out(p, n);
#pragma unroll
        for (int i = 0; i < T::TM; ++i)
#pragma unroll
            for (int r = 0; r < 16; ++r) {
                const int m = m0 + wm_off + i * 32 + mfma_row(r, lane);
                if (m < M) out.store(p, m, acc[i][j][r]);
            }
    }
}

template <int BM, class Loader, bool X3 = false>
__global__ __launch_bounds__(IG_THREADS, (BM == 128 ? (X3 ? 2 : 3) : 1)) void igemm_fwd_kernel(
    typename Loader::Params p, const float* __restrict__ A, int Mp, int Kp, int M, long long N,
    int n_tiles, int m_tiles) {
    igemm_fwd_body<BM, Loader, X3, false>(p, A, Mp, Kp, M, N, n_tiles, m_tiles);
}
template <int BM, class Loader>
__global__ __launch_bounds__(IG_THREADS, (BM == 128 ? 3 : 1)) void igemm_fwd_splitk_kernel(
    typename Loader::Params p, const float* __restrict__ A, int Mp, int Kp, int M, long long N,
    int n_tiles, int m_tiles, float* __restrict__ slab, int split_k) {
    igemm_fwd_body<BM, Loader, false, true>(p, A, Mp, Kp, M, N, n_tiles, m_tiles, slab, split_k);
}
constexpr int SK_ROWS = 8;
template <class Loader>
__global__ __launch_bounds__(256) void splitk_reduce_kernel(typename Loader::Params p, const float* __restrict__ slab, int Z,
                                                            int Mp, long long Np, int M, long long N) {
    const long long n = (long long)blockIdx.x * 256 + threadIdx.x;
    if (n >= N) return;
    typename Loader::Out out(p, n);
    const int m_end = ((int)blockIdx.y + 1) * SK_ROWS < M ? ((int)blockIdx.y + 1) * SK_ROWS : M;
    for (int m = blockIdx.y * SK_ROWS; m < m_end; ++m) {
        float v = 0.0f;
        for (int z = 0; z < Z; ++z) v += slab[((size_t)z * Mp + m) * Np + n];
        out.store(p, m, v);
    }
}

template <int BM, class Loader, int KC, bool SPLITK = false>
__device__ __forceinline__ void igemm_fwd_ws_body(
    const typename Loader::Params& p, const float* __restrict__ A, int Mp, int Kp, int M, long long N,
    int n_tiles, int m_tiles, float* __restrict__ slab = nullptr, int split_k = 0) {
    using T = IgTile<BM>;
    const int kb = SPLITK ? (int)blockIdx.y * split_k : 0;
    const int ke = SPLITK ? (kb + split_k < Kp ? kb + split_k : Kp) : Kp;
    constexpr int LDS_AB = 2 * KC * BM + 2 * KC * IG_BN;
    static_assert(LDS_AB >= 4 * IG_EPI_WAVE, "the operand buffers hold the epilogue staging tiles");
    __shared__ __attribute__((aligned(16))) float smem[LDS_AB];
    float (*As)[KC * BM] = reinterpret_cast<float (*)[KC * BM]>(smem);
    float (*Bs)[KC * IG_BN] = reinterpret_cast<float (*)[KC * IG_BN]>(smem + 2 * KC * BM);
    const bool producer = threadIdx.x >= IG_THREADS;
    const int tid = threadIdx.x & (IG_THREADS - 1), lane = tid & 63, wid = tid >> 6;
    const int wg = xcd_remap(blockIdx.x, n_tiles * m_tiles);
    const int m0 = (wg % m_tiles) * BM;
    const long long n0 = (long long)(wg / m_tiles) * IG_BN;
    if (producer) {
        const int nl = tid & (IG_BN - 1), ksub = tid >> 7;
        Loader ld(p, n0 + nl, n0 + nl < N);
        if constexpr (Loader::kHasSideOutput) { if (m0 != 0) ld.disable_col(); }
        static_assert(!Loader::kHasSideOutput, "two-phase loaders keep per-chunk state (the current tap's weights)");
        constexpr int NH = KC / IG_BK;
        struct Regs {
            f32x4 ra[ig_a_per<BM, KC>()];
            float rb[NH][8];
            typename IgRaw<Loader, Loader::kHasSideOutput>::type raw[NH];
        };
        Regs r0;
        const IgABuf<BM, KC> abuf(A, Mp, Kp, m0, tid);
        auto stage_store = [&](int buf, Regs& r) {
            ig_store_a<BM, KC>(As[buf], tid, r.ra);
#pragma unroll
            for (int h = 0; h < NH; ++h) {
                if constexpr (Loader::kHasSideOutput) ld.finish(r.raw[h], r.rb[h]);
#pragma unroll
                for (int j = 0; j < 8; ++j) Bs[buf][(h * IG_BK + ksub + 2 * j) * IG_BN + nl] = r.rb[h][j];
            }
        };
        auto stage_load = [&](int k0, Regs& r) {
            abuf.load(k0, r.ra);
#pragma unroll
            for (int h = 0; h < NH; ++h) {
                if constexpr (Loader::kHasSideOutput) ld.load_raw(k0 + h * IG_BK, ksub, r.raw[h]);
                else ld.load(k0 + h * IG_BK, ksub, r.rb[h]);
            }
        };
        stage_load(kb, r0);
        stage_store(0, r0);
        if (kb + KC < ke) stage_load(kb + KC, r0);
        __syncthreads();
        int c1 = 0;
        for (int k0 = kb; k0 < ke; k0 += KC) {
            if (k0 + KC < ke) {
                stage_store(c1 ^ 1, r0);
                if (k0 + 2 * KC < ke) stage_load(k0 + 2 * KC, r0);
            }
            __syncthreads();
            c1 ^= 1;
        }
        return;
    }
    const int wm_off = (wid / T::WN) * (T::TM * 32), wn_off = (wid % T::WN) * (T::TN * 32);
    f32x16 acc[T::TM][T::TN];
#pragma unroll
    for (int i = 0; i < T::TM; ++i)
#pragma unroll
        for (int j = 0; j < T::TN; ++j)
#pragma unroll
            for (int r = 0; r < 16; ++r) acc[i][j][r] = 0.0f;
    __syncthreads();
    int cur = 0;
#ifdef IG_FOLD
    f32x16 tot[T::TM][T::TN];
#pragma unroll
    for (int i = 0; i < T::TM; ++i)
#pragma unroll
        for (int j = 0; j < T::TN; ++j)
#pragma unroll
            for (int r = 0; r < 16; ++r) tot[i][j][r] = 0.0f;
    int since = 0;
#endif
    for (int k0 = kb; k0 < ke; k0 += KC) {
        ig_mma_chunk<BM, KC>(As[cur], Bs[cur], acc, wm_off, wn_off, lane);
#ifdef IG_FOLD
        if (++since == IG_FOLD) {
            since = 0;
#pragma unroll
            for (int i = 0; i < T::TM; ++i)
#pragma unroll
                for (int j = 0; j < T::TN; ++j)
#pragma unroll
                    for (int r = 0; r < 16; ++r) { tot[i][j][r] += acc[i][j][r]; acc[i][j][r] = 0.0f; }
        }
#endif
        __syncthreads();
        cur ^= 1;
    }
#ifdef IG_FOLD
#pragma unroll
    for (int i = 0; i < T::TM; ++i)
#pragma unroll
        for (int j = 0; j < T::TN; ++j)
#pragma unroll
            for (int r = 0; r < 16; ++r) acc[i][j][r] += tot[i][j][r];
#endif
    if constexpr (SPLITK) {
        ig_store_slab<BM>(slab, acc, Mp, (long long)n_tiles * IG_BN, m0, n0, wm_off, wn_off, lane);
        return;
    }
    if constexpr (IgHasQuads<typename Loader::Out>::value) {
        ig_epilogue_quads<BM, Loader>(p, acc, m0, n0, wm_off, wn_off, lane, M, N);
        return;
    }
    if constexpr (Loader::Out::kVec4) {
// ... 112 lines not shown
        }
        f32x16 acc[T::TM][T::TN];
#pragma unroll
        for (int i = 0; i < T::TM; ++i)
#pragma unroll
            for (int j = 0; j < T::TN; ++j)
#pragma unroll
                for (int r = 0; r < 16; ++r) acc[i][j][r] = 0.0f;
#pragma unroll
        for (int c = 0; c < KP / IG_KC; ++c)
            ig_mma_chunk<BM>(As + c * IG_KC * BM, Bs + c * IG_KC * IG_BN, acc, wm_off, wn_off, lane);
        if constexpr (IgHasQuads<typename Loader::Out>::value) {
            ig_epilogue_quads<BM, Loader>(p, acc, m0, n0, wm_off, wn_off, lane, M, N);
        } else {
        __syncthreads();
        if (Loader::Out::vec4_ok(p)) {
            ig_epilogue_vec4<BM, Loader>(p, As + wid * IG_EPI_WAVE, acc, m0, n0, wm_off, wn_off, lane, M, N);
        } else {
#pragma unroll
            for (int j = 0; j < T::TN; ++j) {
                const long long n = n0 + wn_off + j * 32 + (lane & 31);
                if (n >= N) continue;
                typename Loader::Out out(p, n);
#pragma unroll
                for (int i = 0; i < T::TM; ++i)
#pragma unroll
                    for (int r = 0; r < 16; ++r) {
                        const int m = m0 + wm_off + i * 32 + mfma_row(r, lane);
                        if (m < M) out.store(p, m, acc[i][j][r]);
                    }
            }
        }
        }
    }
}

constexpr int WG_BM = 64, WG_BJ = 64, WG_BP = 32;

struct IgPixelCursor {
    int left_;
    int b_, pp_, oy_, ox_;
    int crossed_;
    bool valid_;
    __device__ __forceinline__ void init(long long n, long long n_end, int HoWo, int Wo) {
        const long long d = n_end - n;
        left_ = d > 0x7fffffffll ? 0x7fffffff : (d < 0 ? 0 : (int)d);
        valid_ = left_ > 0;
        const long long nn = valid_ ? n : 0;
        b_ = (int)(nn / HoWo);
        pp_ = (int)(nn - (long long)b_ * HoWo);
        oy_ = pp_ / Wo;
        ox_ = pp_ - oy_ * Wo;
        crossed_ = 0;
    }
    __device__ __forceinline__ void advance(int HoWo, int Wo) {
        left_ = left_ > WG_BP ? left_ - WG_BP : 0;
        valid_ = left_ > 0;
        pp_ += WG_BP;
        ox_ += WG_BP;
        crossed_ = 0;
        while (ox_ >= Wo) { ox_ -= Wo; ++oy_; }
        while (pp_ >= HoWo) { pp_ -= HoWo; ++b_; ++crossed_; oy_ = pp_ / Wo; ox_ = pp_ - oy_ * Wo; }
    }
};
__device__ __forceinline__ int ig_mad24(int a, int b, int c) { return __mul24(a, b) + c; }
template <int NV, int STEP>
__device__ __forceinline__ void ig_buf_rows(buf_rsrc rs, const IgPixelCursor& c, unsigned image_base, int HoWo, int row0,
                                            int sub, float (&v)[NV]) {
    const unsigned voff = c.valid_ ? image_base + (unsigned)ig_mad24(sub, HoWo, c.pp_) * 4u : IG_BUF_OOB;
#pragma unroll
    for (int i = 0; i < NV; ++i) v[i] = ig_buf_load(rs, voff, (unsigned)((row0 + STEP * i) * HoWo) * (unsigned)sizeof(float));
}

template <int NG, int STEP>
__device__ __forceinline__ void ig_wgrad_store_bias(float (&bs)[NG], float* __restrict__ dst, int pl, int sub) {
    static_assert(WG_BP == 32, "a row group's pixel lanes are one half of a wave");
#pragma unroll
    for (int i = 0; i < NG; ++i) {
        float v = bs[i];
#pragma unroll
        for (int d = 16; d >= 1; d >>= 1) v += __shfl_xor(v, d, 64);
        if (pl == 0) dst[sub + STEP * i] = v;
    }
}

template <class WLoader, int BM, int BJ>
__global__ __launch_bounds__(IG_THREADS) void igemm_wgrad_kernel(
    typename WLoader::Params p, float* __restrict__ slabs, int Mp, int Jp, long long N, long long pix_per_split,
    float* __restrict__ bslab) {
    constexpr int GLD = BM + 1, BLD = BJ + 1;
    constexpr int STEP = IG_THREADS / WG_BP;
    constexpr int TM = (BM == 128 && BJ == 128) ? 2 : 1, TJ = (BM / 32) * (BJ / 32) / 4 / TM;
    constexpr int WJ = BJ / 32 / TJ, NG = BM / STEP, NB = BJ / STEP;
    static_assert((BM / 32 / TM) * WJ == 4, "four waves tile the block");
    __shared__ float Gs[2][WG_BP * GLD];
    __shared__ float Bs[2][WG_BP * BLD];
    const int tid = threadIdx.x, lane = tid & 63, wid = tid >> 6;
    const int j0 = blockIdx.x * BJ, m0 = blockIdx.y * BM;
    const long long n_begin = (long long)blockIdx.z * pix_per_split;
    long long n_end = n_begin + pix_per_split;
    if (n_end > N) n_end = N;
    const int pl = tid % WG_BP, sub = tid / WG_BP;
    const int wm_off = (wid / WJ) * 32 * TM, wj_off = (wid % WJ) * 32 * TJ;
    WLoader ld(p, n_begin + pl, n_end);
    f32x16 acc[TM][TJ];
#pragma unroll
    for (int i = 0; i < TM; ++i)
#pragma unroll
        for (int t = 0; t < TJ; ++t)
#pragma unroll
            for (int r = 0; r < 16; ++r) acc[i][t][r] = 0.0f;
    float rg[NG], rb[NB];
    const bool do_bias = bslab != nullptr && blockIdx.x == 0;
    float bs[NG];
#pragma unroll
    for (int i = 0; i < NG; ++i) bs[i] = 0.0f;
    auto stage_store = [&](int buf) {
#pragma unroll
        for (int i = 0; i < NG; ++i) Gs[buf][pl * GLD + sub + STEP * i] = rg[i];
#pragma unroll
        for (int i = 0; i < NB; ++i) Bs[buf][pl * BLD + sub + STEP * i] = rb[i];
        if (do_bias) {
#pragma unroll
            for (int i = 0; i < NG; ++i) bs[i] += rg[i];
        }
    };
    auto stage_load = [&]() {
        ld.template load_g<NG, STEP>(m0, sub, rg);
        ld.template load_b<NB, STEP>(j0, sub, rb);
    };
    stage_load();
    stage_store(0);
    if (n_begin + WG_BP < n_end) { ld.advance(); stage_load(); }
    __syncthreads();
    int cur = 0;
    const int kl = lane >> 5, il = lane & 31;
    for (long long nb = n_begin; nb < n_end; nb += WG_BP) {
        {
            const float* gp = Gs[cur] + kl * GLD + wm_off + il;
            const float* bp = Bs[cur] + kl * BLD + wj_off + il;
            float a[2][2][TM], b[2][2][TJ];
            auto frag = [&](int kk, float (&fa)[2][TM], float (&fb)[2][TJ]) {
#pragma unroll
                for (int i = 0; i < TM; ++i) { fa[0][i] = gp[kk * GLD + i * 32]; fa[1][i] = gp[(kk + 2) * GLD + i * 32]; }
#pragma unroll
                for (int t = 0; t < TJ; ++t) { fb[0][t] = bp[kk * BLD + t * 32]; fb[1][t] = bp[(kk + 2) * BLD + t * 32]; }
            };
            auto mma = [&](const float (&fa)[2][TM], const float (&fb)[2][TJ]) {
#pragma unroll
                for (int h = 0; h < 2; ++h)
#pragma unroll
                    for (int i = 0; i < TM; ++i)
#pragma unroll
                        for (int t = 0; t < TJ; ++t)
                            acc[i][t] = __builtin_amdgcn_mfma_f32_32x32x2f32(fa[h][i], fb[h][t], acc[i][t], 0, 0, 0);
            };
            frag(0, a[0], b[0]);
#pragma unroll
            for (int kk = 0; kk < WG_BP; kk += 8) {
                frag(kk + 4, a[1], b[1]);
                __builtin_amdgcn_sched_barrier(0);
                mma(a[0], b[0]);
                __builtin_amdgcn_sched_barrier(0);
                if (kk + 8 < WG_BP) frag(kk + 8, a[0], b[0]);
                __builtin_amdgcn_sched_barrier(0);
                mma(a[1], b[1]);
                __builtin_amdgcn_sched_barrier(0);
            }
        }
        if (nb + WG_BP < n_end) {
            stage_store(cur ^ 1);
            if (nb + 2 * WG_BP < n_end) { ld.advance(); stage_load(); }
        }
        __syncthreads();
        cur ^= 1;
    }
    float* slab = slabs + (size_t)blockIdx.z * Mp * Jp;
#pragma unroll
    for (int i = 0; i < TM; ++i)
#pragma unroll
        for (int t = 0; t < TJ; ++t)
#pragma unroll
            for (int r = 0; r < 16; ++r) {
                const int m = m0 + wm_off + i * 32 + mfma_row(r, lane);
                const int j = j0 + wj_off + t * 32 + (lane & 31);
                slab[(size_t)m * Jp + j] = acc[i][t][r];
            }
    if (do_bias) ig_wgrad_store_bias<NG, STEP>(bs, bslab + (size_t)blockIdx.z * Mp + m0, pl, sub);
}

template <class WLoader, int BM, int BJ>
__global__ __launch_bounds__(2 * IG_THREADS) void igemm_wgrad_ws_kernel(
    typename WLoader::Params p, float* __restrict__ slabs, int Mp, int Jp, long long N, long long pix_per_split,
    float* __restrict__ bslab) {
    constexpr int GLD = BM + 1, BLD = BJ + 1;
    constexpr int STEP = IG_THREADS / WG_BP;
    constexpr int TM = (BM == 128 && BJ == 128) ? 2 : 1, TJ = (BM / 32) * (BJ / 32) / 4 / TM;
    constexpr int WJ = BJ / 32 / TJ, NG = BM / STEP, NB = BJ / STEP;
    static_assert((BM / 32 / TM) * WJ == 4, "four waves tile the block");
    __shared__ float Gs[2][WG_BP * GLD];
    __shared__ float Bs[2][WG_BP * BLD];
    const bool producer = threadIdx.x >= IG_THREADS;
    const int tid = threadIdx.x & (IG_THREADS - 1), lane = tid & 63, wid = tid >> 6;
    const int j0 = blockIdx.x * BJ, m0 = blockIdx.y * BM;
    const long long n_begin = (long long)blockIdx.z * pix_per_split;
    long long n_end = n_begin + pix_per_split;
    if (n_end > N) n_end = N;
    if (producer) {
        const int pl = tid % WG_BP, sub = tid / WG_BP;
        WLoader ld(p, n_begin + pl, n_end);
        struct Regs { float rg[NG], rb[NB]; };
        const bool do_bias = bslab != nullptr && blockIdx.x == 0;
        float bs[NG];
#pragma unroll
        for (int i = 0; i < NG; ++i) bs[i] = 0.0f;
        auto stage_store = [&](int buf, const Regs& r) {
#pragma unroll
            for (int i = 0; i < NG; ++i) Gs[buf][pl * GLD + sub + STEP * i] = r.rg[i];
#pragma unroll
            for (int i = 0; i < NB; ++i) Bs[buf][pl * BLD + sub + STEP * i] = r.rb[i];
            if (do_bias) {
#pragma unroll
                for (int i = 0; i < NG; ++i) bs[i] += r.rg[i];
            }
        };
        auto stage_load = [&](Regs& r) {
            ld.template load_g<NG, STEP>(m0, sub, r.rg);
            ld.template load_b<NB, STEP>(j0, sub, r.rb);
        };
        const int nchunk = (int)((n_end - n_begin + WG_BP - 1) / WG_BP);
        Regs r0;
        stage_load(r0);
        stage_store(0, r0);
        if (1 < nchunk) { ld.advance(); stage_load(r0); }
        __syncthreads();
        int cur = 0;
        for (int c = 0; c < nchunk; ++c) {
            if (c + 1 < nchunk) {
                stage_store(cur ^ 1, r0);
                if (c + 2 < nchunk) { ld.advance(); stage_load(r0); }
            }
            __syncthreads();
            cur ^= 1;
        }
        if (do_bias) ig_wgrad_store_bias<NG, STEP>(bs, bslab + (size_t)blockIdx.z * Mp + m0, pl, sub);
        return;
    }
    const int wm_off = (wid / WJ) * 32 * TM, wj_off = (wid % WJ) * 32 * TJ;
    f32x16 acc[TM][TJ];
#pragma unroll
    for (int i = 0; i < TM; ++i)
#pragma unroll
        for (int t = 0; t < TJ; ++t)
#pragma unroll
            for (int r = 0; r < 16; ++r) acc[i][t][r] = 0.0f;
    __syncthreads();
    int cur = 0;
    const int kl = lane >> 5, il = lane & 31;
    for (long long nb = n_begin; nb < n_end; nb += WG_BP) {
        const float* gp = Gs[cur] + kl * GLD + wm_off + il;
        const float* bp = Bs[cur] + kl * BLD + wj_off + il;
        float a[2][2][TM], b[2][2][TJ];
        auto frag = [&](int kk, float (&fa)[2][TM], float (&fb)[2][TJ]) {
#pragma unroll
            for (int i = 0; i < TM; ++i) { fa[0][i] = gp[kk * GLD + i * 32]; fa[1][i] = gp[(kk + 2) * GLD + i * 32]; }
#pragma unroll
            for (int t = 0; t < TJ; ++t) { fb[0][t] = bp[kk * BLD + t * 32]; fb[1][t] = bp[(kk + 2) * BLD + t * 32]; }
        };
        auto mma = [&](const float (&fa)[2][TM], const float (&fb)[2][TJ]) {
#pragma unroll
            for (int h = 0; h < 2; ++h)
#pragma unroll
                for (int i = 0; i < TM; ++i)
#pragma unroll
                    for (int t = 0; t < TJ; ++t)
                        acc[i][t] = __builtin_amdgcn_mfma_f32_32x32x2f32(fa[h][i], fb[h][t], acc[i][t], 0, 0, 0);
        };
        frag(0, a[0], b[0]);
#pragma unroll
        for (int kk = 0; kk < WG_BP; kk += 8) {
            frag(kk + 4, a[1], b[1]);
            __builtin_amdgcn_sched_barrier(0);
            mma(a[0], b[0]);
            __builtin_amdgcn_sched_barrier(0);
            if (kk + 8 < WG_BP) frag(kk + 8, a[0], b[0]);
            __builtin_amdgcn_sched_barrier(0);
            mma(a[1], b[1]);
            __builtin_amdgcn_sched_barrier(0);
        }
        __syncthreads();
        cur ^= 1;
    }
    float* slab = slabs + (size_t)blockIdx.z * Mp * Jp;
#pragma unroll
    for (int i = 0; i < TM; ++i)
#pragma unroll
        for (int t = 0; t < TJ; ++t)
#pragma unroll
            for (int r = 0; r < 16; ++r) {
// ... 8 lines not shown
```

centernet-uda_amd/hip_runtime/__init__.py:

```python
import ctypes
import os
import threading
import weakref

import torch

_PKG_ROOT = os.path.dirname(os.path.dirname(os.path.abspath(__file__)))
LIB_PATH = os.path.join(_PKG_ROOT, 'libcenternet_uda_hip.so')
ABI_VERSION = 2

_lib = None
_lock = threading.Lock()
_workspaces = {}

c_int, c_size_t, c_void_p, c_float = ctypes.c_int, ctypes.c_size_t, ctypes.c_void_p, ctypes.c_float


def lib():
    global _lib
    if _lib is None:
        with _lock:
            if _lib is None:
                if not os.path.exists(LIB_PATH):
                    raise RuntimeError(
                        "%s not found: build it with `make -C centernet-uda_amd/csrc` "
                        "(or __graft_entry__.build()); there is no CPU/eager fallback" % LIB_PATH)
                l = ctypes.CDLL(LIB_PATH)
                l.cnuda_last_error.restype = ctypes.c_char_p
                l.cnuda_abi_version.restype = c_int
                if l.cnuda_abi_version() != ABI_VERSION:
                    raise RuntimeError("libcenternet_uda_hip.so ABI %d != expected %d"
                                       % (l.cnuda_abi_version(), ABI_VERSION))
                for name in dir(_Sig):
                    if name.startswith('cnuda_'):
                        restype, argtypes = getattr(_Sig, name)
                        fn = getattr(l, name)
                        fn.restype, fn.argtypes = restype, argtypes
                _lib = l
    return _lib


_I = c_int
_P = c_void_p


_LL = ctypes.c_longlong
_F = c_float
_WS = [_P, c_size_t, _P]


class _Sig:
    cnuda_decode_workspace_bytes = (c_size_t, [_I] * 5)
    cnuda_decode_set_max_bands = (_I, [_I])
    cnuda_decode_set_stage2_threads = (_I, [_I])
    cnuda_decode_detection = (_I, [_P] * 5 + [_I] * 8 + _WS)
    cnuda_nms = (_I, [_P, _P] + [_I] * 5 + [_P])
    cnuda_dcn_v2_workspace_bytes = (c_size_t, [_I] * 14)
    cnuda_dcn_v2_forward = (_I, [_P] * 6 + [_I] * 14 + _WS)
    cnuda_dcn_v2_backward = (_I, [_P] * 11 + [_I] * 14 + _WS)
    cnuda_dcn_v2_forward_cols = (_I, [_P] * 7 + [_I] * 14 + _WS)
    cnuda_dcn_v2_forward_act = (_I, [_P] * 7 + [_F] + [_I] * 14 + _WS)
    cnuda_dcn_v2_forward_stats = (_I, [_P] * 8 + [_I] * 16 + _WS)
    cnuda_dcn_v2_stats_block = (_I, [_I] * 14 + [_P])
    cnuda_dcn_v2_forward_om = (_I, [_P] * 7 + [_I] * 2 + [_F] + [_I] * 14 + _WS)
    cnuda_dcn_v2_backward_om = (_I, [_P] * 7 + [_I] + [_P] * 3 + [_I] * 14 + _WS)
    cnuda_dcn_v2_backward_cols = (_I, [_P] * 12 + [_I] * 14 + _WS)
    cnuda_dcn_v2_backward_acc = (_I, [_P] * 8 + [_I] + [_P] * 4 + [_I] * 14 + _WS)
    cnuda_dcn_v2_psroi_pooling_workspace_bytes = (c_size_t, [_I] * 4)
    cnuda_dcn_v2_psroi_pooling_forward = (_I, [_P] * 5 + [_I] * 6 + [_F] + [_I] * 5 + [_F, _I, _P])
    cnuda_dcn_v2_psroi_pooling_backward = (_I, [_P] * 6 + [_I, _P] + [_I] * 6 + [_F] + [_I] * 5 + [_F, _I] + _WS)
    cnuda_conv2d_workspace_bytes = (c_size_t, [_I] * 11)
    cnuda_conv2d_forward = (_I, [_P] * 4 + [_I] * 11 + [_F] + _WS)
    cnuda_conv2d_forward_res = (_I, [_P] * 5 + [_I] * 11 + [_F] + _WS)
    cnuda_conv2d_rowsig_supported = (_I, [_I] * 11)
    cnuda_conv2d_forward_rowsig = (_I, [_P] * 4 + [_I] * 12 + _WS)
    cnuda_conv2d_rowquads_supported = (_I, [_I] * 11)
    cnuda_conv2d_cat_supported = (_I, [_P, _I, _I, _I, _I, _I])
    cnuda_conv2d_cat_forward = (_I, [_P, _P, _I, _P, _P, _P, _P, _F, _I, _I, _I, _I] + _WS)
    cnuda_conv2d_cat_backward_data = (_I, [_P, _P, _P, _P, _P, _P, _I, _I, _I, _I, _I] + _WS)
    cnuda_conv2d_cat_backward_weight = (_I, [_P, _P, _I, _P, _P, _I, _I, _I, _I] + _WS)
    cnuda_conv2d_forward_rowquads = (_I, [_P] * 3 + [_I] * 11 + _WS)
    cnuda_conv2d_backward_data = (_I, [_P] * 3 + [_I] * 11 + _WS)
    cnuda_conv2d_backward_data_add = (_I, [_P] * 5 + [_I] * 11 + _WS)
    cnuda_conv2d_stats_block = (_I, [_I] * 11 + [_P, _P])
    cnuda_conv2d_forward_stats = (_I, [_P] * 6 + [_I] * 11 + [_F] + _WS)
    cnuda_bn_train_forward_stats = (_I, [_P, _P, _LL, _I] + [_P] * 9 + [_F, _F, _I, _I, _I, _LL, _I] + _WS)
    cnuda_conv2d_backward_weight = (_I, [_P] * 4 + [_I] * 11 + _WS)
    cnuda_conv2d_norm_input_supported = (_I, [_I] * 11)
    cnuda_conv2d_forward_norm_input = (_I, [_P] * 5 + [_I] + [_P] * 4 + [_I] * 11 + [_F] + _WS)
    cnuda_conv2d_backward_weight_norm_input = (_I, [_P] * 5 + [_I] + [_P] * 3 + [_I] * 11 + _WS)
    cnuda_bn_workspace_bytes = (c_size_t, [_I, _I, _LL])
    cnuda_bn_train_forward = (_I, [_P] * 10 + [_F, _F, _I, _I, _I, _LL, _I] + _WS)
    cnuda_bn_eval_forward = (_I, [_P] * 7 + [_F, _I, _I, _I, _LL, _P])
    cnuda_bn_backward = (_I, [_P] * 11 + [_I, _I, _I, _LL, _I] + _WS)
    cnuda_maxpool2d_forward = (_I, [_P] * 2 + [_I] * 5 + [_P])
    cnuda_maxpool2d_backward = (_I, [_P] * 3 + [_I] * 5 + [_P])
    cnuda_maxpool2d_backward_acc = (_I, [_P] * 3 + [_I] * 6 + [_P])
    cnuda_maxpool2d_window_forward = (_I, [_P] * 2 + [_I] * 7 + [_P])
    cnuda_maxpool2d_window_backward = (_I, [_P] * 3 + [_I] * 7 + [_P])
    cnuda_dwconvt2d_forward = (_I, [_P] * 3 + [_I] * 7 + [_P])
    cnuda_dwconvt2d_add_forward = (_I, [_P] * 4 + [_I] * 7 + [_P])
    cnuda_dwconvt2d_workspace_bytes = (c_size_t, [_I] * 3)
    cnuda_dwconvt2d_backward = (_I, [_P] * 5 + [_I] * 7 + _WS)
    cnuda_dwconv2d_workspace_bytes = (c_size_t, [_I] * 3)
    cnuda_dwconv2d_forward = (_I, [_P] * 3 + [_I] * 7 + [_P])
    cnuda_dwconv2d_backward = (_I, [_P] * 5 + [_I] * 7 + _WS)
    cnuda_dwconv2d_same_workspace_bytes = (c_size_t, [_I] * 3)
    cnuda_dwconv2d_same_forward = (_I, [_P] * 3 + [_I] * 10 + [_P])
    cnuda_dwconv2d_same_backward = (_I, [_P] * 5 + [_I] * 10 + _WS)
    cnuda_swish_forward = (_I, [_P] * 2 + [_LL, _P])
    cnuda_swish_backward = (_I, [_P] * 3 + [_LL, _P])
    cnuda_se_workspace_bytes = (c_size_t, [_I] * 3)
    cnuda_se_forward = (_I, [_P] * 9 + [_I] * 3 + [_LL, _P])
    cnuda_se_backward = (_I, [_P] * 12 + [_I] * 3 + [_LL] + _WS)
    cnuda_drop_connect_add = (_I, [_P] * 4 + [_I, _LL, _P])
    cnuda_pad_right_bottom = (_I, [_P] * 2 + [_LL] + [_I] * 4 + [_P])
    cnuda_add = (_I, [_P] * 3 + [_LL, _P])
    cnuda_act_backward = (_I, [_P] * 3 + [_LL, _F, _P])
    cnuda_conv1x1_backward_data_act = (_I, [_P] * 4 + [_I] * 3 + [_LL, _F, _P])
    cnuda_copy_channels = (_I, [_P, _P, _I, _I, _LL, _I, _I, _I, _I, _P])
    cnuda_split_offset_mask = (_I, [_P] * 3 + [_I, _I, _LL, _P])
    cnuda_split_offset_mask_backward = (_I, [_P] * 4 + [_I, _I, _LL, _P])
    cnuda_loss_workspace_bytes = (c_size_t, [])
    cnuda_focal_loss_forward = (_I, [_P] * 4 + [_LL, _F] + _WS)
    cnuda_focal_loss_backward = (_I, [_P] * 5 + [_LL, _F, _P])
    cnuda_reg_l1_forward = (_I, [_P] * 5 + [_I, _I, _I, _LL, _I, _F, _F, _P])
    cnuda_reg_l1_backward = (_I, [_P] * 7 + [_I, _I, _I, _LL, _I, _F, _F, _P])
    cnuda_kps_l1_forward = (_I, [_P] * 6 + [_I, _I, _I, _LL, _I, _I, _F, _F, _P])
    cnuda_kps_l1_backward = (_I, [_P] * 8 + [_I, _I, _I, _LL, _I, _I, _F, _F, _P])
    cnuda_decode_keypoints = (_I, [_P] * 4 + [_I] * 5 + [_P])
    cnuda_softmax_loss_forward = (_I, [_P, _P, _I, _I, _LL, _I] + _WS)
    cnuda_softmax_loss_backward = (_I, [_P] * 3 + [_I, _I, _LL, _I, _P])
    cnuda_entropy_map_forward = (_I, [_P, _P, _I, _I, _LL, _P])
    cnuda_entropy_map_backward = (_I, [_P] * 3 + [_I, _I, _LL, _P])
    cnuda_entropy_eta_loss_forward = (_I, [_P, _P, _I, _I, _LL, _F] + _WS)
    cnuda_entropy_eta_loss_backward = (_I, [_P] * 3 + [_I, _I, _LL, _F, _P])
    cnuda_bce_const_forward = (_I, [_P, _F, _P, _LL, _P])
    cnuda_bce_const_backward = (_I, [_P, _F, _P, _P, _LL, _P])
    cnuda_sigmoid_clamp_ = (_I, [_P, _P, _LL, _P])
    cnuda_gather_feat = (_I, [_P] * 3 + [_I, _I, _I, _LL, _P])
    cnuda_encode_targets = (_I, [_P] * 10 + [_I] * 5 + [_P])
    cnuda_fda_workspace_bytes = (c_size_t, [_I] * 4)
    cnuda_fda_source_to_target = (_I, [_P] * 4 + [_I] * 4 + _WS)
    cnuda_adam_step = (_I, [_P] * 4 + [_LL] + [_F] * 5 + [_I, _P])
    cnuda_set_matrix_mode = (_I, [_I])
    cnuda_get_matrix_mode = (_I, [])
    cnuda_pack_cache_attach = (_I, [_P, c_size_t])
    cnuda_pack_stamp = (_I, [ctypes.c_ulonglong, ctypes.c_ulonglong])
    cnuda_pack_refresh = (_I, [_P, ctypes.c_size_t, ctypes.c_ulonglong, ctypes.c_ulonglong, _P, ctypes.c_size_t, _P])
    cnuda_pack_cache_used = (c_size_t, [])
    cnuda_pack_cache_fills = (ctypes.c_ulonglong, [])
    cnuda_pack_cache_resets = (ctypes.c_ulonglong, [])
    cnuda_prof_enable = (_I, [_I])
    cnuda_prof_arm = (_I, [_I])
    cnuda_prof_collect = (_I, [_P, _P, _P, _I])
    cnuda_prof_name_len = (_I, [])
    cnuda_launch_log_enable = (_I, [_I])
    cnuda_launch_log_collect = (_I, [ctypes.c_char_p, c_size_t])
    cnuda_dcn_set_fused_min_tiles = (_I, [_I])
    cnuda_dcn_set_scatter_margin = (_I, [_I])
    cnuda_dcn_set_offset_regime = (_I, [_I])
    cnuda_dcn_set_walk_tile = (_I, [_I])
    cnuda_dcn_offset_census = (_I, [_P, _I, _I, _LL, _P, _P])
    cnuda_conv_set_halo_policy = (_I, [_I, _I])
    cnuda_conv_set_splitk_policy = (_I, [_I])


_PARAM_EPOCH = 0


def bump_param_epoch(rewritten=None):
# ... 310 lines not shown
```

centernet-uda_amd/hip_runtime/ops.py:

```python
import ctypes

import torch
from torch.autograd import Function
from torch.autograd.function import once_differentiable

from . import check, f32c, lib, pack_stamp, prof_arm, ptr, require_gpu, stats_side_output, stream, workspace
from .arena import grad_sink
from .fanout import accumulate_in_place, accumulate_target, claim, first_writer, slot_of


def _pair(v):
    return tuple(v) if isinstance(v, (tuple, list)) else (v, v)


def _ws(nbytes, like):
    w = workspace(nbytes, like.device)
    return ptr(w), w.numel()


def _param_grad(param, needed=True):
    if not needed or param is None:
        return None, None
    v = grad_sink(param)
    if v is not None:
# ... 33 lines not shown
            if norm is not None:
                xr, mean, invstd, gamma, beta, ipg = norm
                check(L.cnuda_conv2d_forward_norm_input(ptr(xr), ptr(mean), ptr(invstd), ptr(gamma), ptr(beta), int(ipg),
                                                        ptr(weight), ptr(bias), ptr(y), ptr(stats), *g, float(act_slope),
                                                        wp, wn, stream()), 'conv2d_forward_norm_input')
            elif sig_from is not None:
                check(L.cnuda_conv2d_forward_rowsig(ptr(x), ptr(weight), ptr(bias), ptr(y), int(sig_from), *g, wp, wn, stream()),
                      'conv2d_forward_rowsig')
            elif stats is None:
                check(L.cnuda_conv2d_forward(ptr(x), ptr(weight), ptr(bias), ptr(y), *g, float(act_slope),
                                             wp, wn, stream()), 'conv2d_forward')
            else:
                check(L.cnuda_conv2d_forward_stats(ptr(x), ptr(weight), ptr(bias), ptr(None), ptr(y), ptr(stats), *g,
                                                   float(act_slope), wp, wn, stream()), 'conv2d_forward_stats')
        ctx.geom, ctx.act_slope, ctx.has_bias, ctx.pack_token = g, act_slope, bias is not None, pack_token
        ctx.norm_ipg = None
        if norm is not None:
            ctx.norm_ipg = int(norm[5])
            ctx.save_for_backward(norm[0], weight, y if act_slope >= 0 else None, bias, norm[1], norm[2], norm[3], norm[4])
        else:
            ctx.save_for_backward(x, weight, y if act_slope >= 0 else None, bias)
        return y

    @staticmethod
    @once_differentiable
    def backward(ctx, gy):
        x, weight, y, bias = ctx.saved_tensors[:4]
        g = ctx.geom
        L = lib()
        gy = f32c(gy)
        if ctx.act_slope >= 0:
            t = torch.empty_like(gy)
            check(L.cnuda_act_backward(ptr(gy), ptr(y), ptr(t), gy.numel(), float(ctx.act_slope), stream()))
            gy = t
        wp, wn = _ws(L.cnuda_conv2d_workspace_bytes(*g), x)
        gx = gw = gb = None
        B, C, H, W, Co, kh, kw = g[:7]
        Ho, Wo = gy.shape[2], gy.shape[3]
        if ctx.needs_input_grad[0]:
            gx, addend, addend2 = accumulate_target(ctx.slot, x)
            prof_arm('conv_dgrad', B, C, H, W, Co, kh, kw, Ho, Wo)
            with pack_stamp(ctx.pack_token, weight):
                check(L.cnuda_conv2d_backward_data_add(ptr(gy), ptr(weight), ptr(addend), ptr(addend2), ptr(gx), *g, wp, wn,
                                                       stream()), 'conv2d_backward_data')
        if ctx.needs_input_grad[1] or (ctx.has_bias and ctx.needs_input_grad[2]):
            gw_buf, gw = _param_grad(weight)
            gb_buf, gb = _param_grad(bias, ctx.has_bias)
            prof_arm('conv_wgrad', B, C, H, W, Co, kh, kw, Ho, Wo)
            if ctx.norm_ipg is not None:
                mean, invstd, gamma, beta = ctx.saved_tensors[4:]
                check(L.cnuda_conv2d_backward_weight_norm_input(ptr(x), ptr(mean), ptr(invstd), ptr(gamma), ptr(beta),
                                                                ctx.norm_ipg, ptr(gy), ptr(gw_buf), ptr(gb_buf), *g, wp, wn,
                                                                stream()), 'conv2d_backward_weight_norm_input')
            else:
                check(L.cnuda_conv2d_backward_weight(ptr(x), ptr(gy), ptr(gw_buf), ptr(gb_buf), *g, wp, wn, stream()),
                      'conv2d_backward_weight')
        return gx, gw, gb, None, None, None, None, None, None, None


def conv2d_rowsig(x, weight, bias, stride, padding, sig_from, pack_token=0):
    g = _conv_geom(x, weight, stride, padding)
    if bias is None or not lib().cnuda_conv2d_rowsig_supported(*g):
        return None
    return _Conv2d.apply(x, weight, bias, stride, padding, -1.0, pack_token, None, None, int(sig_from))


EPILOGUE_STATS = True


def with_bn_stats(emit, call):
    if not (emit and EPILOGUE_STATS):
        return call(None)
    box = []
    y = call(box)
    if box:
        y._cnuda_bn_stats = box[0]
    return y


def conv2d(x, weight, bias=None, stride=1, padding=0, act_slope=-1.0, pack_token=0, emit_stats=False):
    norm = getattr(x, '_cnuda_deferred_bn', None)
    if norm is not None:
        g = _conv_geom(x, weight, stride, padding)
        if not lib().cnuda_conv2d_norm_input_supported(*g):
            raise RuntimeError("conv2d: the input is a deferred BatchNorm output, but no apply-on-load kernel takes this "
                               "convolution (cnuda_conv2d_norm_input_supported); ask batch_norm_act to apply it")
    return with_bn_stats(emit_stats, lambda box: _Conv2d.apply(x, weight, bias, stride, padding, float(act_slope), pack_token,
                                                               box, norm, None))


class _ConvActConv1x1(Function):

    @staticmethod
    def forward(ctx, x, w1, b1, w2, b2, padding, act_slope, token1, token2, lead=None):
        require_gpu(x, w1, b1, w2, b2)
        ctx.slot, ctx.full = slot_of(x), None
        if lead is not None and lead < x.shape[0]:
            ctx.full = x.shape
            x = f32c(x)[:lead]
        x, w1, w2 = f32c(x), f32c(w1), f32c(w2)
        b1 = None if b1 is None else f32c(b1)
        b2 = None if b2 is None else f32c(b2)
        g1 = _conv_geom(x, w1, 1, padding)
        B, C, H, W, Ch, kh, kw, sh, sw, ph, pw = g1
        Ho, Wo = H + 2 * ph - kh + 1, W + 2 * pw - kw + 1
        hidden = torch.empty((B, Ch, Ho, Wo), dtype=torch.float32, device=x.device)
        L = lib()
        wp, wn = _ws(L.cnuda_conv2d_workspace_bytes(*g1), x)
        prof_arm('conv_fwd', B, C, H, W, Ch, kh, kw, Ho, Wo)
        with pack_stamp(token1, w1):
            check(L.cnuda_conv2d_forward(ptr(x), ptr(w1), ptr(b1), ptr(hidden), *g1, float(act_slope), wp, wn, stream()),
                  'conv2d_forward')
        g2 = _conv_geom(hidden, w2, 1, 0)
        Co = g2[4]
        y = torch.empty((B, Co, Ho, Wo), dtype=torch.float32, device=x.device)
        wp, wn = _ws(L.cnuda_conv2d_workspace_bytes(*g2), x)
        prof_arm('conv_fwd', B, Ch, Ho, Wo, Co, 1, 1, Ho, Wo)
        with pack_stamp(token2, w2):
            check(L.cnuda_conv2d_forward(ptr(hidden), ptr(w2), ptr(b2), ptr(y), *g2, -1.0, wp, wn, stream()),
                  'conv2d_forward')
        ctx.g1, ctx.g2, ctx.act_slope, ctx.token1 = g1, g2, float(act_slope), token1
        ctx.has_b1, ctx.has_b2 = b1 is not None, b2 is not None
        ctx.save_for_backward(x, w1, b1, w2, b2, hidden)
        return y

    @staticmethod
    @once_differentiable
    def backward(ctx, gy):
        x, w1, b1, w2, b2, hidden = ctx.saved_tensors
        g1, g2 = ctx.g1, ctx.g2
        L = lib()
        gy = f32c(gy)
        if gy.data_ptr() % 16:
            gy = gy.clone()
        B, C, H, W, Ch, kh, kw = g1[:7]
        Co, Ho, Wo = g2[4], hidden.shape[2], hidden.shape[3]
        gx = gw1 = gb1 = gw2 = gb2 = None
        if ctx.needs_input_grad[3] or (ctx.has_b2 and ctx.needs_input_grad[4]):
            gw2_buf, gw2 = _param_grad(w2)
            gb2_buf, gb2 = _param_grad(b2, ctx.has_b2)
            wp, wn = _ws(L.cnuda_conv2d_workspace_bytes(*g2), x)
            prof_arm('conv_wgrad', B, Ch, Ho, Wo, Co, 1, 1, Ho, Wo)
            check(L.cnuda_conv2d_backward_weight(ptr(hidden), ptr(gy), ptr(gw2_buf), ptr(gb2_buf), *g2, wp, wn, stream()),
                  'conv2d_backward_weight')
        gh = torch.empty_like(hidden)
        check(L.cnuda_conv1x1_backward_data_act(ptr(gy), ptr(w2), ptr(hidden), ptr(gh), B, Co, Ch, Ho * Wo,
                                                ctx.act_slope, stream()), 'conv1x1_backward_data_act')
        wp, wn = _ws(L.cnuda_conv2d_workspace_bytes(*g1), x)
        if ctx.needs_input_grad[0]:
            prof_arm('conv_dgrad', B, C, H, W, Ch, kh, kw, Ho, Wo)
            slot = ctx.slot
            if ctx.full is None:
                gx, addend, addend2 = accumulate_target(slot, x)
                part = gx
            elif (gx := accumulate_in_place(slot)) is not None:
                part = addend = gx[:B]
                addend2 = None
            else:
                gx = claim(slot, torch.empty(ctx.full, dtype=torch.float32, device=x.device))
                gx[B:].zero_()
                part, addend, addend2 = gx[:B], None, None
            with pack_stamp(ctx.token1, w1):
                check(L.cnuda_conv2d_backward_data_add(ptr(gh), ptr(w1), ptr(addend), ptr(addend2), ptr(part), *g1, wp, wn,
                                                       stream()), 'conv2d_backward_data')
        if ctx.needs_input_grad[1] or (ctx.has_b1 and ctx.needs_input_grad[2]):
            gw1_buf, gw1 = _param_grad(w1)
            gb1_buf, gb1 = _param_grad(b1, ctx.has_b1)
            prof_arm('conv_wgrad', B, C, H, W, Ch, kh, kw, Ho, Wo)
            check(L.cnuda_conv2d_backward_weight(ptr(x), ptr(gh), ptr(gw1_buf), ptr(gb1_buf), *g1, wp, wn, stream()),
# ... 986 lines not shown
```

include/centernet_uda_hip.h:

```cpp
#ifndef CENTERNET_UDA_HIP_H
#define CENTERNET_UDA_HIP_H

#include <stddef.h>
#include <stdint.h>

#ifdef __cplusplus
extern "C" {
#endif

#define CNUDA_ERR_INVALID_ARGUMENT (-1)
#define CNUDA_ABI_VERSION 2

typedef void* cnuda_stream_t;

int cnuda_abi_version(void);
const char* cnuda_last_error(void);

int cnuda_set_matrix_mode(int mode);
int cnuda_get_matrix_mode(void);

int cnuda_pack_cache_attach(void* arena, size_t bytes);
int cnuda_pack_stamp(unsigned long long token, unsigned long long version);
size_t cnuda_pack_cache_used(void);
unsigned long long cnuda_pack_cache_fills(void);
// ... 65 lines not shown
int cnuda_dcn_v2_backward_om(const float* input, const float* weight, const float* bias, const float* om,
                             const float* grad_output, const float* columns, float* grad_input, int accumulate_input,
                             float* grad_om, float* grad_weight, float* grad_bias,
                             int B, int C, int H, int W, int Cout, int kh, int kw, int sh, int sw, int ph, int pw,
                             int dh, int dw, int dg, void* workspace, size_t workspace_bytes, cnuda_stream_t stream);

int cnuda_dcn_v2_forward_cols(const float* input, const float* weight, const float* bias,
                              const float* offset, const float* mask, float* output, float* columns,
                              int B, int C, int H, int W, int Cout, int kh, int kw,
                              int sh, int sw, int ph, int pw, int dh, int dw, int dg,
                              void* workspace, size_t workspace_bytes, cnuda_stream_t stream);
int cnuda_dcn_v2_backward_cols(const float* input, const float* weight, const float* bias,
                               const float* offset, const float* mask, const float* grad_output,
                               const float* columns,
                               float* grad_input, float* grad_offset, float* grad_mask,
                               float* grad_weight, float* grad_bias,
                               int B, int C, int H, int W, int Cout, int kh, int kw,
                               int sh, int sw, int ph, int pw, int dh, int dw, int dg,
                               void* workspace, size_t workspace_bytes, cnuda_stream_t stream);

int cnuda_dcn_v2_backward_acc(const float* input, const float* weight, const float* bias,
                              const float* offset, const float* mask, const float* grad_output,
                              const float* columns,
                              float* grad_input, int accumulate_input, float* grad_offset, float* grad_mask,
                              float* grad_weight, float* grad_bias,
                              int B, int C, int H, int W, int Cout, int kh, int kw,
                              int sh, int sw, int ph, int pw, int dh, int dw, int dg,
                              void* workspace, size_t workspace_bytes, cnuda_stream_t stream);

size_t cnuda_dcn_v2_psroi_pooling_workspace_bytes(int B, int num_rois, int output_dim, int pooled_size);
int cnuda_dcn_v2_psroi_pooling_forward(const float* input, const float* rois, const float* trans,
                                       float* output, float* output_count,
                                       int B, int channels, int H, int W, int num_rois, int no_trans,
                                       float spatial_scale, int output_dim, int group_size, int pooled_size,
                                       int part_size, int sample_per_part, float trans_std, int num_classes,
                                       cnuda_stream_t stream);
int cnuda_dcn_v2_psroi_pooling_backward(const float* grad_output, const float* input, const float* rois,
                                        const float* trans, const float* output_count,
                                        float* grad_input, int accumulate_input, float* grad_trans,
                                        int B, int channels, int H, int W, int num_rois, int no_trans,
                                        float spatial_scale, int output_dim, int group_size, int pooled_size,
                                        int part_size, int sample_per_part, float trans_std, int num_classes,
                                        void* workspace, size_t workspace_bytes, cnuda_stream_t stream);

size_t cnuda_conv2d_workspace_bytes(int B, int C, int H, int W, int Cout, int kh, int kw,
                                    int sh, int sw, int ph, int pw);
int cnuda_conv2d_forward(const float* x, const float* weight, const float* bias, float* y,
                         int B, int C, int H, int W, int Cout, int kh, int kw,
                         int sh, int sw, int ph, int pw, float act_slope,
                         void* workspace, size_t workspace_bytes, cnuda_stream_t stream);
int cnuda_conv2d_forward_res(const float* x, const float* weight, const float* bias, const float* residual, float* y,
                             int B, int C, int H, int W, int Cout, int kh, int kw,
                             int sh, int sw, int ph, int pw, float act_slope,
                             void* workspace, size_t workspace_bytes, cnuda_stream_t stream);
int cnuda_conv2d_rowsig_supported(int B, int C, int H, int W, int Cout, int kh, int kw, int sh, int sw, int ph, int pw);
int cnuda_conv2d_forward_rowsig(const float* x, const float* weight, const float* bias, float* y, int sig_from,
                                int B, int C, int H, int W, int Cout, int kh, int kw, int sh, int sw, int ph, int pw,
                                void* workspace, size_t workspace_bytes, cnuda_stream_t stream);
int cnuda_conv2d_cat_supported(const int* cs, int n, int B, int H, int W, int Cout);
int cnuda_conv2d_cat_forward(const float* const* xs, const int* cs, int n, const float* weight, const float* bias ,
                             float* y, float* stats, float act_slope ,
                             int B, int H, int W, int Cout, void* workspace, size_t workspace_bytes, cnuda_stream_t stream);
int cnuda_conv2d_cat_backward_data(const float* grad_y, const float* weight, float* const* grad_xs, const float* const* adds,
                                   const float* const* add2s, const int* cs, int n, int B, int H, int W, int Cout,
                                   void* workspace, size_t workspace_bytes, cnuda_stream_t stream);
int cnuda_conv2d_cat_backward_weight(const float* const* xs, const int* cs, int n, const float* grad_y, float* grad_weight,
                                     int B, int H, int W, int Cout, void* workspace, size_t workspace_bytes,
                                     cnuda_stream_t stream);
int cnuda_conv2d_rowquads_supported(int B, int C, int H, int W, int Cout, int kh, int kw, int sh, int sw, int ph, int pw);
int cnuda_conv2d_forward_rowquads(const float* x, const float* weight, float* y,
                                  int B, int C, int H, int W, int Cout, int kh, int kw, int sh, int sw, int ph, int pw,
                                  void* workspace, size_t workspace_bytes, cnuda_stream_t stream);
int cnuda_conv2d_stats_block(int B, int C, int H, int W, int Cout, int kh, int kw, int sh, int sw, int ph, int pw, int* rows,
                             int* blocks_per_image );
int cnuda_conv2d_forward_stats(const float* x, const float* weight, const float* bias, const float* residual, float* y,
                               float* stats, int B, int C, int H, int W, int Cout, int kh, int kw,
                               int sh, int sw, int ph, int pw, float act_slope,
                               void* workspace, size_t workspace_bytes, cnuda_stream_t stream);
int cnuda_conv2d_backward_data(const float* grad_y, const float* weight, float* grad_x,
                               int B, int C, int H, int W, int Cout, int kh, int kw,
                               int sh, int sw, int ph, int pw,
                               void* workspace, size_t workspace_bytes, cnuda_stream_t stream);
int cnuda_conv2d_norm_input_supported(int B, int C, int H, int W, int Cout, int kh, int kw, int sh, int sw, int ph, int pw);
int cnuda_conv2d_forward_norm_input(const float* x, const float* mean, const float* invstd, const float* gamma,
                                    const float* beta, int imgs_per_group, const float* weight, const float* bias, float* y,
                                    float* stats, int B, int C, int H, int W, int Cout, int kh, int kw, int sh, int sw, int ph,
                                    int pw, float act_slope, void* workspace, size_t workspace_bytes, cnuda_stream_t stream);
int cnuda_conv2d_backward_weight_norm_input(const float* x, const float* mean, const float* invstd, const float* gamma,
                                            const float* beta, int imgs_per_group, const float* grad_y, float* grad_weight,
                                            float* grad_bias, int B, int C, int H, int W, int Cout, int kh, int kw, int sh,
                                            int sw, int ph, int pw, void* workspace, size_t workspace_bytes,
                                            cnuda_stream_t stream);
int cnuda_conv2d_backward_data_add(const float* grad_y, const float* weight, const float* addend, const float* addend2,
                                   float* grad_x,
                                   int B, int C, int H, int W, int Cout, int kh, int kw,
                                   int sh, int sw, int ph, int pw,
                                   void* workspace, size_t workspace_bytes, cnuda_stream_t stream);
int cnuda_conv2d_backward_weight(const float* x, const float* grad_y, float* grad_weight, float* grad_bias,
                                 int B, int C, int H, int W, int Cout, int kh, int kw,
                                 int sh, int sw, int ph, int pw,
                                 void* workspace, size_t workspace_bytes, cnuda_stream_t stream);

size_t cnuda_bn_workspace_bytes(int B, int C, long long HW);
int cnuda_bn_train_forward(const float* x, const float* gamma, const float* beta, const float* residual,
                           float* y, float* save_mean, float* save_invstd,
                           float* running_mean, float* running_var,
                           long long* num_batches_tracked ,
                           float momentum, float eps, int relu,
                           int B, int C, long long HW,
                           int groups ,
                           void* workspace, size_t workspace_bytes, cnuda_stream_t stream);
int cnuda_bn_train_forward_stats(const float* x, const float* stats, long long blocks_per_group, int rows, const float* gamma,
                                 const float* beta, const float* residual, float* y, float* save_mean, float* save_invstd,
                                 float* running_mean, float* running_var, long long* num_batches_tracked,
                                 float momentum, float eps, int relu, int B, int C, long long HW, int groups,
                                 void* workspace, size_t workspace_bytes, cnuda_stream_t stream);
int cnuda_bn_eval_forward(const float* x, const float* gamma, const float* beta,
                          const float* running_mean, const float* running_var, const float* residual,
                          float* y, float eps, int relu, int B, int C, long long HW, cnuda_stream_t stream);
int cnuda_bn_backward(const float* grad_y, const float* x, const float* y, const float* gamma,
                      const float* beta ,
                      const float* save_mean, const float* save_invstd,
                      float* grad_x, float* grad_residual, float* grad_gamma, float* grad_beta,
                      int relu, int B, int C, long long HW, int groups,
                      void* workspace, size_t workspace_bytes, cnuda_stream_t stream);

int cnuda_maxpool2d_forward(const float* x, float* y, int B, int C, int H, int W, int k, cnuda_stream_t stream);
int cnuda_maxpool2d_backward(const float* x, const float* grad_y, float* grad_x,
                             int B, int C, int H, int W, int k, cnuda_stream_t stream);
int cnuda_maxpool2d_backward_acc(const float* x, const float* grad_y, float* grad_x, int accumulate, int B, int C, int H, int W,
                                 int k, cnuda_stream_t stream);
int cnuda_maxpool2d_window_forward(const float* x, float* y, int B, int C, int H, int W, int k, int s, int p,
                                   cnuda_stream_t stream);
int cnuda_maxpool2d_window_backward(const float* x, const float* grad_y, float* grad_x,
                                    int B, int C, int H, int W, int k, int s, int p, cnuda_stream_t stream);
int cnuda_dwconvt2d_forward(const float* x, const float* w, float* y,
                            int B, int C, int H, int W, int k, int s, int p, cnuda_stream_t stream);
int cnuda_dwconvt2d_add_forward(const float* x, const float* w, const float* skip, float* y,
                                int B, int C, int H, int W, int k, int s, int p, cnuda_stream_t stream);
size_t cnuda_dwconvt2d_workspace_bytes(int B, int C, int k);
int cnuda_dwconvt2d_backward(const float* x, const float* w, const float* grad_y, float* grad_x, float* grad_w,
                             int B, int C, int H, int W, int k, int s, int p,
                             void* workspace, size_t workspace_bytes, cnuda_stream_t stream);
size_t cnuda_dwconv2d_workspace_bytes(int B, int C, int k);
int cnuda_dwconv2d_forward(const float* x, const float* w, float* y, int B, int C, int H, int W, int k, int s, int p,
                           cnuda_stream_t stream);
int cnuda_dwconv2d_backward(const float* x, const float* w, const float* grad_y, float* grad_x, float* grad_w,
                            int B, int C, int H, int W, int k, int s, int p,
                            void* workspace, size_t workspace_bytes, cnuda_stream_t stream);
int cnuda_add(const float* a, const float* b, float* out, long long n, cnuda_stream_t stream);
int cnuda_act_backward(const float* grad_y, const float* y, float* grad_x, long long n, float slope,
                       cnuda_stream_t stream);
int cnuda_conv1x1_backward_data_act(const float* grad_y, const float* weight, const float* hidden, float* grad_hidden,
                                    int B, int Co, int Ch, long long HW, float slope, cnuda_stream_t stream);
int cnuda_copy_channels(const float* src, float* dst, int B, int Cn, long long HW,
                        int Csrc, int src_off, int Cdst, int dst_off, cnuda_stream_t stream);
int cnuda_split_offset_mask(const float* om, float* offset, float* mask, int B, int taps, long long HW,
                            cnuda_stream_t stream);
int cnuda_split_offset_mask_backward(const float* grad_offset, const float* grad_mask, const float* mask,
                                     float* grad_om, int B, int taps, long long HW, cnuda_stream_t stream);

size_t cnuda_loss_workspace_bytes(void);
int cnuda_focal_loss_forward(const float* logits, const float* gt, float* prob, float* out2, long long n,
                             float weight, void* workspace, size_t workspace_bytes, cnuda_stream_t stream);
int cnuda_focal_loss_backward(const float* logits, const float* gt, const float* out2, const float* upstream,
                              float* grad_logits, long long n, float weight, cnuda_stream_t stream);
// ... 71 lines not shown
```

Before: 212.0 images/sec.

## Defer BasicBlock bn1 apply into implicit-GEMM conv loaders for forward and wgrad

Extends the BatchNorm+ReLU apply-on-load path from the small-channel kernels to the implicit-GEMM forward and weight-gradient kernels. Each block fills a shared-memory scale/shift table per group and channel, and the loaders normalise input values as they stage them. BasicBlock now sets defer_apply on bn1 in training whenever the second conv's geometry supports it. The goal is to skip writing and re-reading the normalised activation tensor. The cost is extra per-element arithmetic, a shared table plus a sync in every block, and more shared-memory pressure.

```diff
diff --git a/centernet-uda_amd/backends/dla.py b/centernet-uda_amd/backends/dla.py
--- a/centernet-uda_amd/backends/dla.py
+++ b/centernet-uda_amd/backends/dla.py
@@ -88,6 +88,16 @@
         return bool(hr.lib().cnuda_conv2d_norm_input_supported(1, cin, 64, 64, cout, k, k, 1, 1, k // 2, k // 2))
     except Exception:
         return False
+
+
+BLOCK_DEFER = os.environ.get('CNUDA_BLOCK_DEFER', '1') != '0'
+
+
+def _block_defers(shape, cout, stride, groups):
+    import hip_runtime as hr
+    h, w = (shape[2] - 1) // stride + 1, (shape[3] - 1) // stride + 1
+    return BLOCK_DEFER and shape[0] % groups == 0 and bool(hr.lib().cnuda_conv2d_norm_input_groups_supported(
+        shape[0], cout, h, w, cout, 3, 3, 1, 1, 1, 1, groups))
 
 
 class ConvBnRelu(nn.Sequential):
@@ -149,6 +159,10 @@
                                     self._fold_gen)
         if residual is None or residual is x:
             x, residual = fork(x, 2)
+        if self.training and x.is_cuda:
+            import hip_runtime as hr
+            self.bn1.defer_apply = _block_defers(x.shape, self.conv2.out_channels, self.conv1.stride[0],
+                                                 int(hr.current_groups()))
         y = self.bn1(self.conv1(x), relu=True)
         return self.bn2(self.conv2(y), residual=residual, relu=True)
 
diff --git a/centernet-uda_amd/csrc/conv.hip b/centernet-uda_amd/csrc/conv.hip
--- a/centernet-uda_amd/csrc/conv.hip
+++ b/centernet-uda_amd/csrc/conv.hip
@@ -20,6 +20,7 @@
     float* y;
     float act_slope;
     const float* residual;
+    IgNorm nrm;
 };
 struct ConvFwdStatsParams : ConvFwdParams {
     float* stats;
@@ -40,6 +41,8 @@
     const float* x_b;
     int iy0, ix0;
     bool valid;
+    int goff = 0, lk0 = 0;
+    static constexpr int kNormTab = FAST ? 0 : 2;
     int ck0 = 0, ctap = 0, cc0 = 0, cr = 0, cs = 0;
     __device__ __forceinline__ void seek(int k0) {
         while (ck0 < k0) {
@@ -56,9 +59,26 @@
         iy0 = oy * g.sh - g.ph;
         ix0 = ox * g.sw - g.pw;
         x_b = p.x + (size_t)b * g.C * g.H * g.W;
+        if (!FAST && p.nrm.mean) goff = b / p.nrm.ipg * g.C;
+    }
+    __device__ __forceinline__ void norm(float (&v)[8], int ksub, const float2* __restrict__ tab) const {
+        const int K = g.kh * g.kw * g.C;
+#pragma unroll
+        for (int j = 0; j < 8; ++j) {
+            const int k = lk0 + ksub + 2 * j;
+            float val = 0.0f;
+            if (valid && k < K) {
+                const int tap = k / g.C, c = k - tap * g.C;
+                const int r = tap / g.kw, s = tap - r * g.kw;
+                const int iy = iy0 + r, ix = ix0 + s;
+                if (iy >= 0 && iy < g.H && ix >= 0 && ix < g.W) val = ig_norm_act(v[j], tab[goff + c]);
+            }
+            v[j] = val;
+        }
     }
     __device__ __forceinline__ void load(int k0, int ksub, float (&v)[8]) {
         const int HW = g.H * g.W, K = g.kh * g.kw * g.C;
+        if (!FAST) lk0 = k0;
         if (FAST) {
             seek(k0);
             const int c0 = cc0 + ksub;
@@ -120,6 +140,8 @@
     buf_rsrc rs;
     unsigned pix_off;
     unsigned tap_ok;
+    int goff;
+    static constexpr int kNormTab = 1;
     int ck0 = 0, ctap = 0, cc0 = 0, cr = 0, cs = 0;
     __device__ __forceinline__ void seek(int k0) {
         while (ck0 < k0) {
@@ -136,6 +158,7 @@
         const int iy0 = oy * g.sh - g.ph, ix0 = ox * g.sw - g.pw;
         rs = ig_make_rsrc(p.x, (unsigned)((size_t)g.B * g.C * g.H * g.W * sizeof(float)));
         pix_off = (unsigned)(((b * g.C * g.H + iy0) * g.W + ix0) * (int)sizeof(float));
+        goff = p.nrm.mean ? b / p.nrm.ipg * g.C : 0;
         tap_ok = 0;
         if (n_valid) {
             for (int r = 0; r < g.kh; ++r)
@@ -143,6 +166,16 @@
                     const int iy = iy0 + r, ix = ix0 + s;
                     if (iy >= 0 && iy < g.H && ix >= 0 && ix < g.W) tap_ok |= 1u << (r * g.kw + s);
                 }
+        }
+    }
+    __device__ __forceinline__ void norm(float (&v)[8], int ksub, const float2* __restrict__ tab) const {
+        const int tap = ctap < 32 ? ctap : 31;
+        const bool ok = ck0 < g.kh * g.kw * g.C && ((tap_ok >> tap) & 1u);
+        const float2* t = tab + goff + cc0 + __builtin_amdgcn_readfirstlane(ksub);
+#pragma unroll
+        for (int j = 0; j < 8; ++j) {
+            const float a = ig_norm_act(v[j], t[2 * j]);
+            v[j] = ok ? a : 0.0f;
         }
     }
     __device__ __forceinline__ void load(int k0, int ksub, float (&v)[8]) {
@@ -162,6 +195,7 @@
 struct ConvFwdBufSigLoader : ConvFwdBufLoader {
     using Params = ConvFwdSigParams;
     static const char* name() { return "ConvFwdBufSigLoader"; }
+    static constexpr int kNormTab = 0;
     __device__ ConvFwdBufSigLoader(const Params& p, long long n, bool n_valid) : ConvFwdBufLoader(p, n, n_valid) {}
     struct Out : ConvFwdLoader<true>::Out {
         __device__ Out(const Params& p, long long n) : ConvFwdLoader<true>::Out(p, n) {}
@@ -183,6 +217,7 @@
 
 struct ConvFwdBufQuadLoader : ConvFwdBufLoader {
     static const char* name() { return "ConvFwdBufQuadLoader"; }
+    static constexpr int kNormTab = 0;
     __device__ ConvFwdBufQuadLoader(const Params& p, long long n, bool n_valid) : ConvFwdBufLoader(p, n, n_valid) {}
     struct Out {
         float* base;
@@ -566,6 +601,7 @@
 struct ConvWParams {
     ConvGeom g;
     const float *x, *gy;
+    IgNorm nrm;
 };
 template <int MODE>
 struct ConvWLoader {
@@ -638,6 +674,8 @@
     buf_rsrc rg, rx;
     IgPixelCursor c;
     unsigned gimg, ximg;
+    int goff;
+    static constexpr int kNormTab = 1;
     __device__ ConvWBufLoader(const Params& pp, long long n, long long n_end) : p(pp) {
         const ConvGeom& g = p.g;
         rg = ig_make_rsrc(p.gy, (unsigned)((size_t)g.B * g.Co * g.Ho * g.Wo * sizeof(float)));
@@ -645,6 +683,7 @@
         c.init(n, n_end, g.Ho * g.Wo, g.Wo);
         gimg = (unsigned)(c.b_ * g.Co * g.Ho * g.Wo) * 4u;
         ximg = (unsigned)(c.b_ * g.C * g.H * g.W) * 4u;
+        goff = p.nrm.mean ? c.b_ / p.nrm.ipg * g.C : 0;
     }
     __device__ __forceinline__ void advance() {
         const ConvGeom& g = p.g;
@@ -652,6 +691,27 @@
         if (c.crossed_) {
             gimg += (unsigned)(c.crossed_ * g.Co * g.Ho * g.Wo) * 4u;
             ximg += (unsigned)(c.crossed_ * g.C * g.H * g.W) * 4u;
+            if (p.nrm.mean) goff = c.b_ / p.nrm.ipg * g.C;
+        }
+    }
+    template <int NV, int STEP>
+    __device__ __forceinline__ void norm_b(int j0, int jsub, float (&v)[NV], const float2* __restrict__ tab) const {
+        const ConvGeom& g = p.g;
+        const int K = g.kh * g.kw * g.C;
+        const int iy0 = ig_mad24(c.oy_, g.sh, -g.ph), ix0 = ig_mad24(c.ox_, g.sw, -g.pw);
+        constexpr int PER = 64 / STEP;
+#pragma unroll
+        for (int h = 0; h < NV / PER; ++h) {
+            const int jg = j0 + 64 * h;
+            const int tap = jg / g.C, c0 = jg - tap * g.C;
+            const int r = tap / g.kw, s = tap - r * g.kw;
+            const bool ok = c.valid_ && jg < K && (unsigned)(iy0 + r) < (unsigned)g.H && (unsigned)(ix0 + s) < (unsigned)g.W;
+            const float2* t = tab + goff + c0 + jsub;
+#pragma unroll
+            for (int i = 0; i < PER; ++i) {
+                const float a = ig_norm_act(v[PER * h + i], t[STEP * i]);
+                v[PER * h + i] = ok ? a : 0.0f;
+            }
         }
     }
     template <int NV, int STEP>
@@ -682,6 +742,21 @@
 
 struct ConvWBufLoaderC8 : ConvWBufLoader {
     static const char* name() { return "ConvWBufLoaderC8"; }
+    template <int NV, int STEP>
+    __device__ __forceinline__ void norm_b(int j0, int jsub, float (&v)[NV], const float2* __restrict__ tab) const {
+        const ConvGeom& g = p.g;
+        const int K = g.kh * g.kw * g.C;
+        const int iy0 = ig_mad24(c.oy_, g.sh, -g.ph), ix0 = ig_mad24(c.ox_, g.sw, -g.pw);
+#pragma unroll
+        for (int i = 0; i < NV; ++i) {
+            const int jg = j0 + STEP * i;
+            const int tap = jg / g.C, c0 = jg - tap * g.C;
+            const int r = tap / g.kw, s = tap - r * g.kw;
+            const bool ok = c.valid_ && jg < K && (unsigned)(iy0 + r) < (unsigned)g.H && (unsigned)(ix0 + s) < (unsigned)g.W;
+            const float a = ig_norm_act(v[i], tab[goff + c0 + jsub]);
+            v[i] = ok ? a : 0.0f;
+        }
+    }
     __device__ ConvWBufLoaderC8(const Params& pp, long long n, long long n_end) : ConvWBufLoader(pp, n, n_end) {}
     template <int NV, int STEP>
     __device__ __forceinline__ void load_b(int j0, int jsub, float (&v)[NV]) {
@@ -971,6 +1046,16 @@
     return q.bmf == 32 ? 32 : 64;
 }
 
+bool igemm_norm_ok(const ConvGeom& g, const ConvPlan& q, int groups) {
+    if (matrix_mode() != 0 || groups <= 0 || g.B % groups != 0) return false;
+    const bool fwd_buf = (q.fwd == FwdPath::Buf || q.fwd == FwdPath::BufSplitK) && q.bmf >= 64 && q.Kpf > 64;
+    if (!fwd_buf && q.fwd != FwdPath::Ptr) return false;
+    if (q.wgrad != WgradPath::Buf && q.wgrad != WgradPath::BufC8) return false;
+    const long long pairs = (long long)groups * g.C;
+    if (pairs > IG_NORM_TAB) return false;
+    return (q.wbm == 128 && q.wbj == 128) ? pairs <= IG_NORM_TAB : (q.wbm == 64 && q.wbj == 64 && pairs <= IG_NORM_TAB / 2);
+}
+
 struct HconvFwd {
     using Params = ConvFwdParams;
     using Out = ConvFwdLoader<true>::Out;
@@ -1175,6 +1260,13 @@
 
 using namespace cnuda;
 
+static int conv_forward(const float* x, const float* weight, const float* bias, const float* residual, float* y, float* stats,
+                        const IgNorm* nrm, int B, int C, int H, int W, int Cout, int kh, int kw, int sh, int sw, int ph, int pw,
+                        float act_slope, void* workspace, size_t workspace_bytes, cnuda_stream_t stream);
+static int conv_backward_weight(const float* x, const float* grad_y, float* grad_weight, float* grad_bias, const IgNorm* nrm,
+                                int B, int C, int H, int W, int Cout, int kh, int kw, int sh, int sw, int ph, int pw,
+                                void* workspace, size_t workspace_bytes, cnuda_stream_t stream);
+
 
 extern "C" int cnuda_conv_set_splitk_policy(int max_tiles) {
     const int prev = g_splitk_max_tiles;
@@ -1221,6 +1313,13 @@
                                           float* y, float* stats, int B, int C, int H, int W, int Cout, int kh, int kw,
                                           int sh, int sw, int ph, int pw, float act_slope, void* workspace,
                                           size_t workspace_bytes, cnuda_stream_t stream) {
+    return conv_forward(x, weight, bias, residual, y, stats, nullptr, B, C, H, W, Cout, kh, kw, sh, sw, ph, pw, act_slope,
+                        workspace, workspace_bytes, stream);
+}
+
+static int conv_forward(const float* x, const float* weight, const float* bias, const float* residual, float* y, float* stats,
+                        const IgNorm* nrm, int B, int C, int H, int W, int Cout, int kh, int kw, int sh, int sw, int ph, int pw,
+                        float act_slope, void* workspace, size_t workspace_bytes, cnuda_stream_t stream) {
     CNUDA_REQUIRE(x && weight && y, "cnuda_conv2d_forward: null pointer");
     ConvGeom g;
     if (int rc = fill_geom(g, B, C, H, W, Cout, kh, kw, sh, sw, ph, pw, "cnuda_conv2d_forward")) return rc;
@@ -1228,13 +1327,19 @@
     CNUDA_REQUIRE(!stats || (!residual && act_slope < 0.0f && plan_stats_block(g, q, nullptr, nullptr) != 0),
                   "cnuda_conv2d_forward_stats: no statistics for this call (cnuda_conv2d_stats_block says which)");
     const FwdPath path = residual ? q.fwd_gemm : q.fwd;
-    if (path == FwdPath::SmallC)
+    if (path == FwdPath::SmallC) {
+        SmallNorm nm{};
+        if (nrm) nm = SmallNorm{nrm->mean, nrm->invstd, nrm->gamma, nrm->beta, nrm->ipg};
         return smallc_forward(x, weight, bias, y, B, C, H, W, Cout, kh, kw, sh, ph, pw, act_slope, 0, workspace,
-                              workspace_bytes, (hipStream_t)stream, stats);
+                              workspace_bytes, (hipStream_t)stream, stats, nrm ? &nm : nullptr);
+    }
+    CNUDA_REQUIRE(!nrm || (path == q.fwd && igemm_norm_ok(g, q, B / nrm->ipg)),
+                  "cnuda_conv2d_forward_norm_input: geometry without an apply-on-load kernel");
     CNUDA_REQUIRE(workspace && workspace_bytes >= q.fwd_bytes, "cnuda_conv2d_forward: workspace too small");
     hipStream_t st = (hipStream_t)stream;
     Carver cv(workspace, workspace_bytes);
     ConvFwdParams p{g, x, bias, y, act_slope, residual};
+    if (nrm) p.nrm = *nrm;
     const float* A = launch_pack(weight, reinterpret_cast<float*>(cv.take<char>(ig_a_bytes(q.Kpf, q.Mpf))), ig_a_bytes(q.Kpf, q.Mpf),
                                  Cout, C, q.T, path == FwdPath::Halo ? PACK_HALO_FWD : PACK_FWD, q.Kpf, q.Mpf, 0, st);
     switch (path) {
@@ -1440,6 +1545,16 @@
                                           workspace_bytes, stream);
 }
 
+extern "C" int cnuda_conv2d_norm_input_groups_supported(int B, int C, int H, int W, int Cout, int kh, int kw, int sh, int sw,
+                                                        int ph, int pw, int groups) {
+    if (ph == (kh - 1) / 2 && pw == (kw - 1) / 2 && smallc_norm_supported(C, Cout, kh, kw, sh, sw)) return 1;
+    ConvGeom g;
+    if (B <= 0 || C <= 0 || H <= 0 || W <= 0 || Cout <= 0 || kh <= 0 || kw <= 0 || sh <= 0 || sw <= 0 || ph < 0 || pw < 0 ||
+        H + 2 * ph < kh || W + 2 * pw < kw)
+        return 0;
+    if (fill_geom(g, B, C, H, W, Cout, kh, kw, sh, sw, ph, pw, "cnuda_conv2d_norm_input_groups_supported")) return 0;
+    return igemm_norm_ok(g, make_plan(g), groups) ? 1 : 0;
+}
 extern "C" int cnuda_conv2d_norm_input_supported(int B, int C, int H, int W, int Cout, int kh, int kw, int sh, int sw, int ph,
                                                  int pw) {
     (void)B; (void)H; (void)W;
@@ -1452,16 +1567,16 @@
                                                size_t workspace_bytes, cnuda_stream_t stream) {
     CNUDA_REQUIRE(x && mean && invstd && gamma && beta && weight && y, "cnuda_conv2d_forward_norm_input: null pointer");
     CNUDA_REQUIRE(imgs_per_group > 0 && B % imgs_per_group == 0, "cnuda_conv2d_forward_norm_input: statistics groups");
-    CNUDA_REQUIRE(cnuda_conv2d_norm_input_supported(B, C, H, W, Cout, kh, kw, sh, sw, ph, pw),
+    CNUDA_REQUIRE(cnuda_conv2d_norm_input_groups_supported(B, C, H, W, Cout, kh, kw, sh, sw, ph, pw, B / imgs_per_group),
                   "cnuda_conv2d_forward_norm_input: geometry without an apply-on-load kernel");
     if (stats) {
         int rows = 0;
         CNUDA_REQUIRE(act_slope < 0.0f && cnuda_conv2d_stats_block(B, C, H, W, Cout, kh, kw, sh, sw, ph, pw, &rows, nullptr) != 0,
                       "cnuda_conv2d_forward_norm_input: no statistics for this call");
     }
-    const SmallNorm nm{mean, invstd, gamma, beta, imgs_per_group};
-    return smallc_forward(x, weight, bias, y, B, C, H, W, Cout, kh, kw, sh, ph, pw, act_slope, 0, workspace, workspace_bytes,
-                          (hipStream_t)stream, stats, &nm);
+    const IgNorm nm{mean, invstd, gamma, beta, imgs_per_group};
+    return conv_forward(x, weight, bias, nullptr, y, stats, &nm, B, C, H, W, Cout, kh, kw, sh, sw, ph, pw, act_slope, workspace,
+                        workspace_bytes, stream);
 }
 extern "C" int cnuda_conv2d_backward_weight_norm_input(const float* x, const float* mean, const float* invstd,
                                                        const float* gamma, const float* beta, int imgs_per_group,
@@ -1471,17 +1586,11 @@
     CNUDA_REQUIRE(x && mean && invstd && gamma && beta && grad_y && grad_weight,
                   "cnuda_conv2d_backward_weight_norm_input: null pointer");
     CNUDA_REQUIRE(imgs_per_group > 0 && B % imgs_per_group == 0, "cnuda_conv2d_backward_weight_norm_input: statistics groups");
-    CNUDA_REQUIRE(cnuda_conv2d_norm_input_supported(B, C, H, W, Cout, kh, kw, sh, sw, ph, pw),
+    CNUDA_REQUIRE(cnuda_conv2d_norm_input_groups_supported(B, C, H, W, Cout, kh, kw, sh, sw, ph, pw, B / imgs_per_group),
                   "cnuda_conv2d_backward_weight_norm_input: geometry without an apply-on-load kernel");
-    ConvGeom g;
-    if (int rc = fill_geom(g, B, C, H, W, Cout, kh, kw, sh, sw, ph, pw, "cnuda_conv2d_backward_weight_norm_input")) return rc;
-    hipStream_t st = (hipStream_t)stream;
-    const SmallNorm nm{mean, invstd, gamma, beta, imgs_per_group};
-    if (int rc = smallc_backward_weight(x, grad_y, grad_weight, B, C, H, W, Cout, kh, kw, sh, ph, pw, workspace, workspace_bytes,
-                                        st, &nm))
-        return rc;
-    if (grad_bias) launch_channel_sum(grad_y, grad_bias, B, Cout, (long long)g.Ho * g.Wo, st);
-    return check_launch("cnuda_conv2d_backward_weight_norm_input");
+    const IgNorm nm{mean, invstd, gamma, beta, imgs_per_group};
+    return conv_backward_weight(x, grad_y, grad_weight, grad_bias, &nm, B, C, H, W, Cout, kh, kw, sh, sw, ph, pw, workspace,
+                                workspace_bytes, stream);
 }
 
 extern "C" int cnuda_conv2d_backward_data_add(const float* grad_y, const float* weight, const float* addend,
@@ -1605,14 +1714,23 @@
                                             int B, int C, int H, int W, int Cout, int kh, int kw, int sh, int sw,
                                             int ph, int pw, void* workspace, size_t workspace_bytes,
                                             cnuda_stream_t stream) {
+    return conv_backward_weight(x, grad_y, grad_weight, grad_bias, nullptr, B, C, H, W, Cout, kh, kw, sh, sw, ph, pw, workspace,
+                                workspace_bytes, stream);
+}
+
+static int conv_backward_weight(const float* x, const float* grad_y, float* grad_weight, float* grad_bias, const IgNorm* nrm,
+                                int B, int C, int H, int W, int Cout, int kh, int kw, int sh, int sw, int ph, int pw,
+                                void* workspace, size_t workspace_bytes, cnuda_stream_t stream) {
     CNUDA_REQUIRE(x && grad_y && grad_weight, "cnuda_conv2d_backward_weight: null pointer");
     ConvGeom g;
     if (int rc = fill_geom(g, B, C, H, W, Cout, kh, kw, sh, sw, ph, pw, "cnuda_conv2d_backward_weight")) return rc;
     const ConvPlan q = make_plan(g);
     hipStream_t st = (hipStream_t)stream;
     if (q.wgrad == WgradPath::SmallC) {
+        SmallNorm nm{};
+        if (nrm) nm = SmallNorm{nrm->mean, nrm->invstd, nrm->gamma, nrm->beta, nrm->ipg};
         if (int rc = smallc_backward_weight(x, grad_y, grad_weight, B, C, H, W, Cout, kh, kw, sh, ph, pw, workspace,
-                                            workspace_bytes, st))
+                                            workspace_bytes, st, nrm ? &nm : nullptr))
             return rc;
         if (grad_bias) launch_channel_sum(grad_y, grad_bias, B, Cout, (long long)g.Ho * g.Wo, st);
         return check_launch("cnuda_conv2d_backward_weight(small)");
@@ -1621,7 +1739,10 @@
     Carver cv(workspace, workspace_bytes);
     float* slabs = cv.take<float>((size_t)q.Z * q.Mpw * q.Jp);
     float* bsl = grad_bias ? cv.take<float>((size_t)q.Z * q.Mpw) : nullptr;
+    CNUDA_REQUIRE(!nrm || igemm_norm_ok(g, q, B / nrm->ipg),
+                  "cnuda_conv2d_backward_weight_norm_input: geometry without an apply-on-load kernel");
     ConvWParams p{g, x, grad_y};
+    if (nrm) p.nrm = *nrm;
     bool found = true, lds_ok = true;
     {
         ProfScope prof(st);
diff --git a/centernet-uda_amd/csrc/igemm.cuh b/centernet-uda_amd/csrc/igemm.cuh
--- a/centernet-uda_amd/csrc/igemm.cuh
+++ b/centernet-uda_amd/csrc/igemm.cuh
@@ -301,6 +301,24 @@
 
 template <class Loader, bool TWO_PHASE> struct IgRaw { struct type {}; };
 template <class Loader> struct IgRaw<Loader, true> { using type = typename Loader::Raw; };
+
+struct IgNorm {
+    const float *mean, *invstd;
+    const float *gamma, *beta;
+    int ipg;
+};
+template <class L, class = void> struct IgNormTabOf { static constexpr int n = 0; };
+template <class L> struct IgNormTabOf<L, std::void_t<decltype(L::kNormTab)>> { static constexpr int n = L::kNormTab; };
+constexpr int IG_NORM_TAB = 1024;
+template <class Loader, int BM> constexpr int ig_norm_tab() { return (IgNormTabOf<Loader>::n > (BM >= 64 ? 0 : 1)) ? IG_NORM_TAB : 0; }
+__device__ __forceinline__ void ig_fill_norm_tab(float2* __restrict__ tab, const IgNorm& nm, int entries, int C, int tid, int nthreads) {
+    for (int e = tid; e < entries; e += nthreads) {
+        const int c = e % C;
+        const float sc = __fmul_rn(nm.invstd[e], nm.gamma[c]);
+        tab[e] = make_float2(sc, __fsub_rn(nm.beta[c], __fmul_rn(nm.mean[e], sc)));
+    }
+}
+__device__ __forceinline__ float ig_norm_act(float x, float2 t) { return fmaxf(__fadd_rn(__fmul_rn(x, t.x), t.y), 0.0f); }
 
 template <int BM>
 __device__ __forceinline__ void ig_store_slab(float* __restrict__ slab, const f32x16 (&acc)[IgTile<BM>::TM][IgTile<BM>::TN],
@@ -338,6 +356,16 @@
     const int nl = tid & (IG_BN - 1), ksub = tid >> 7;
     Loader ld(p, n0 + nl, n0 + nl < N);
     if constexpr (Loader::kHasSideOutput) { if (m0 != 0) ld.disable_col(); }
+    constexpr int NT = ig_norm_tab<Loader, BM>();
+    const float2* ntab = nullptr;
+    if constexpr (NT > 0) {
+        __shared__ float2 norm_tab[NT];
+        if (p.nrm.mean) {
+            ig_fill_norm_tab(norm_tab, p.nrm, p.g.B / p.nrm.ipg * p.g.C, p.g.C, tid, IG_THREADS);
+            __syncthreads();
+            ntab = norm_tab;
+        }
+    }
 
     f32x16 acc[T::TM][T::TN];
 #pragma unroll
@@ -359,6 +387,10 @@
         if constexpr (Loader::kHasSideOutput) {
 #pragma unroll
             for (int h = 0; h < NH; ++h) ld.finish(raw[h], rb[h]);
+        }
+        if constexpr (NT > 0) {
+            static_assert(NH == 1, "apply on load reads the cursor of the one loader call per chunk");
+            if (ntab) ld.norm(rb[0], ksub, ntab);
         }
         if constexpr (X3) {
             static_assert(NH == 1, "X3 stages one 16-deep MFMA step per chunk");
@@ -531,6 +563,16 @@
     const int wg = xcd_remap(blockIdx.x, n_tiles * m_tiles);
     const int m0 = (wg % m_tiles) * BM;
     const long long n0 = (long long)(wg / m_tiles) * IG_BN;
+    constexpr int NT = (KC == IG_BK) ? ig_norm_tab<Loader, BM>() : 0;
+    const float2* ntab = nullptr;
+    if constexpr (NT > 0) {
+        __shared__ float2 norm_tab[NT];
+        if (p.nrm.mean) {
+            ig_fill_norm_tab(norm_tab, p.nrm, p.g.B / p.nrm.ipg * p.g.C, p.g.C, (int)threadIdx.x, 2 * IG_THREADS);
+            __syncthreads();
+            ntab = norm_tab;
+        }
+    }
     if (producer) {
         const int nl = tid & (IG_BN - 1), ksub = tid >> 7;
         Loader ld(p, n0 + nl, n0 + nl < N);
@@ -546,6 +588,7 @@
         const IgABuf<BM, KC> abuf(A, Mp, Kp, m0, tid);
         auto stage_store = [&](int buf, Regs& r) {
             ig_store_a<BM, KC>(As[buf], tid, r.ra);
+            if constexpr (NT > 0) { if (ntab) ld.norm(r.rb[0], ksub, ntab); }
 #pragma unroll
             for (int h = 0; h < NH; ++h) {
                 if constexpr (Loader::kHasSideOutput) ld.finish(r.raw[h], r.rb[h]);
@@ -824,6 +867,10 @@
         for (int d = 16; d >= 1; d >>= 1) v += __shfl_xor(v, d, 64);
         if (pl == 0) dst[sub + STEP * i] = v;
     }
+}
+
+template <class WLoader, int BM, int BJ> constexpr int ig_wnorm_tab() {
+    return IgNormTabOf<WLoader>::n == 0 ? 0 : ((BM == 128 && BJ == 128) ? IG_NORM_TAB : ((BM == 64 && BJ == 64) ? IG_NORM_TAB / 2 : 0));
 }
 
 template <class WLoader, int BM, int BJ>
@@ -845,6 +892,16 @@
     const int pl = tid % WG_BP, sub = tid / WG_BP;
     const int wm_off = (wid / WJ) * 32 * TM, wj_off = (wid % WJ) * 32 * TJ;
     WLoader ld(p, n_begin + pl, n_end);
+    constexpr int NT = ig_wnorm_tab<WLoader, BM, BJ>();
+    const float2* ntab = nullptr;
+    if constexpr (NT > 0) {
+        __shared__ float2 norm_tab[NT];
+        if (p.nrm.mean) {
+            ig_fill_norm_tab(norm_tab, p.nrm, p.g.B / p.nrm.ipg * p.g.C, p.g.C, tid, IG_THREADS);
+            __syncthreads();
+            ntab = norm_tab;
+        }
+    }
     f32x16 acc[TM][TJ];
 #pragma unroll
     for (int i = 0; i < TM; ++i)
@@ -858,6 +915,7 @@
 #pragma unroll
     for (int i = 0; i < NG; ++i) bs[i] = 0.0f;
     auto stage_store = [&](int buf) {
+        if constexpr (NT > 0) { if (ntab) ld.template norm_b<NB, STEP>(j0, sub, rb, ntab); }
 #pragma unroll
         for (int i = 0; i < NG; ++i) Gs[buf][pl * GLD + sub + STEP * i] = rg[i];
 #pragma unroll
@@ -948,6 +1006,16 @@
     const long long n_begin = (long long)blockIdx.z * pix_per_split;
     long long n_end = n_begin + pix_per_split;
     if (n_end > N) n_end = N;
+    constexpr int NT = ig_wnorm_tab<WLoader, BM, BJ>();
+    const float2* ntab = nullptr;
+    if constexpr (NT > 0) {
+        __shared__ float2 norm_tab[NT];
+        if (p.nrm.mean) {
+            ig_fill_norm_tab(norm_tab, p.nrm, p.g.B / p.nrm.ipg * p.g.C, p.g.C, (int)threadIdx.x, 2 * IG_THREADS);
+            __syncthreads();
+            ntab = norm_tab;
+        }
+    }
     if (producer) {
         const int pl = tid % WG_BP, sub = tid / WG_BP;
         WLoader ld(p, n_begin + pl, n_end);
@@ -956,7 +1024,8 @@
         float bs[NG];
 #pragma unroll
         for (int i = 0; i < NG; ++i) bs[i] = 0.0f;
-        auto stage_store = [&](int buf, const Regs& r) {
+        auto stage_store = [&](int buf, Regs& r) {
+            if constexpr (NT > 0) { if (ntab) ld.template norm_b<NB, STEP>(j0, sub, r.rb, ntab); }
 #pragma unroll
             for (int i = 0; i < NG; ++i) Gs[buf][pl * GLD + sub + STEP * i] = r.rg[i];
 #pragma unroll
diff --git a/centernet-uda_amd/hip_runtime/__init__.py b/centernet-uda_amd/hip_runtime/__init__.py
--- a/centernet-uda_amd/hip_runtime/__init__.py
+++ b/centernet-uda_amd/hip_runtime/__init__.py
@@ -87,6 +87,7 @@
     cnuda_bn_train_forward_stats = (_I, [_P, _P, _LL, _I] + [_P] * 9 + [_F, _F, _I, _I, _I, _LL, _I] + _WS)
     cnuda_conv2d_backward_weight = (_I, [_P] * 4 + [_I] * 11 + _WS)
     cnuda_conv2d_norm_input_supported = (_I, [_I] * 11)
+    cnuda_conv2d_norm_input_groups_supported = (_I, [_I] * 12)
     cnuda_conv2d_forward_norm_input = (_I, [_P] * 5 + [_I] + [_P] * 4 + [_I] * 11 + [_F] + _WS)
     cnuda_conv2d_backward_weight_norm_input = (_I, [_P] * 5 + [_I] + [_P] * 3 + [_I] * 11 + _WS)
     cnuda_bn_workspace_bytes = (c_size_t, [_I, _I, _LL])
diff --git a/centernet-uda_amd/hip_runtime/ops.py b/centernet-uda_amd/hip_runtime/ops.py
--- a/centernet-uda_amd/hip_runtime/ops.py
+++ b/centernet-uda_amd/hip_runtime/ops.py
@@ -139,9 +139,9 @@
     norm = getattr(x, '_cnuda_deferred_bn', None)
     if norm is not None:
         g = _conv_geom(x, weight, stride, padding)
-        if not lib().cnuda_conv2d_norm_input_supported(*g):
+        if not lib().cnuda_conv2d_norm_input_groups_supported(*g, g[0] // int(norm[5])):
             raise RuntimeError("conv2d: the input is a deferred BatchNorm output, but no apply-on-load kernel takes this "
-                               "convolution (cnuda_conv2d_norm_input_supported); ask batch_norm_act to apply it")
+                               "convolution (cnuda_conv2d_norm_input_groups_supported); ask batch_norm_act to apply it")
     return with_bn_stats(emit_stats, lambda box: _Conv2d.apply(x, weight, bias, stride, padding, float(act_slope), pack_token,
                                                                box, norm, None))
 
diff --git a/include/centernet_uda_hip.h b/include/centernet_uda_hip.h
--- a/include/centernet_uda_hip.h
+++ b/include/centernet_uda_hip.h
@@ -171,6 +171,8 @@
                                int sh, int sw, int ph, int pw,
                                void* workspace, size_t workspace_bytes, cnuda_stream_t stream);
 int cnuda_conv2d_norm_input_supported(int B, int C, int H, int W, int Cout, int kh, int kw, int sh, int sw, int ph, int pw);
+int cnuda_conv2d_norm_input_groups_supported(int B, int C, int H, int W, int Cout, int kh, int kw, int sh, int sw, int ph,
+                                             int pw, int groups);
 int cnuda_conv2d_forward_norm_input(const float* x, const float* mean, const float* invstd, const float* gamma,
                                     const float* beta, int imgs_per_group, const float* weight, const float* bias, float* y,
                                     float* stats, int B, int C, int H, int W, int Cout, int kh, int kw, int sh, int sw, int ph,
```

Result: slower. 209.6 images/sec (-1.1%).
